# patngnw/NewsRecommendation

Measured on AMD Instinct MI355X. Metric: train impressions/sec @ batch 512, NRMS, higher is better.
Workload: dtype bf16; 1 GPU; NRMS train step (fwd+bwd+Adam), MIND-small shapes: title_len=30, history=50, npratio=4, 300-d word table; per_gpu_batch=512, global_batch=512, vocab_rows=30000, freeze_embedding=False, compact_history=False, dense_batch=False, feed=resident, deterministic=False, optimizer=flat bucket + HIP fused Adam, parallelism=dp1

## Files before the change

include/nrhip.h:

```cpp
#ifndef NRHIP_H
#define NRHIP_H

#include <stddef.h>
#include <stdint.h>

#ifdef __cplusplus
extern "C" {
#endif

#define NR_F32 0
#define NR_BF16 1

#define NR_OK 0
#define NR_ERR_ARG 1
#define NR_ERR_HIP 2

#define NR_SRC_DENSE 0
#define NR_SRC_GATHER 1

typedef void* nr_stream_t;

int nr_version(void);
int nr_last_error(char* buf, size_t n);
int nr_abi_sizes(size_t* out, int n);
int nr_set_deterministic(void* scratch, size_t bytes);
int nr_set_option(const char* name, int value);
int nr_get_option(const char* name);


int nr_cast_pad(const float* src, int rows, int cols, int ld_src, void* dst, int ld_dst, int dtype,
                int transpose, nr_stream_t stream);
#define NR_CAST_BATCH_MAX 16
typedef struct {
  const float* src;
  void* dst;
  int rows, cols, ld_src, ld_dst, transpose;
} nr_cast_job;
int nr_cast_pad_batch(const nr_cast_job* jobs, int n, int dtype, nr_stream_t stream);
int nr_pack_conv_w(const float* w, int N, int D, void* dst, int Dp, int dtype, nr_stream_t stream);
int nr_unpack_conv_dw(const float* dw_pack, int N, int D, int Dp, float* dw, int accumulate, nr_stream_t stream);
int nr_pack_conv_w_t(const float* w, int N, int D, void* dst, int ld, int dtype, nr_stream_t stream);

int nr_embed_gather_fwd(const void* table, int ld_table, int dtype, const int32_t* ids, int n_ids,
                        int ids_stride, int cols, float* out, int ld_out, nr_stream_t stream);
int nr_embed_gather_bwd(const float* dout, int ld_dout, const int32_t* ids, int n_ids, int ids_stride,
                        int cols, float* dtable, int ld_dtable, nr_stream_t stream);
int nr_gather_cast_fwd(const float* table, int ld_table, const int32_t* ids, int n_ids, int cols, void* out, int ld_out,
                       int out_dtype, nr_stream_t stream);

typedef struct {
  int n, L, d_model, heads, d_head, dtype;
  int src_kind;
  const void* x;
  int ldx;
  const int32_t* ids;
  float p_in;
  uint32_t seed_in;
  float p_out;
  uint32_t seed_out;
  const float* mask;
  const void* w_qkv;
  int ldw;
  const float* b_qkv;
  void* x_rows;
  int ld_rows;
  int32_t* row_ws;
  size_t row_ws_bytes;
  int table_rows;
  const void* proj_table;
  const int32_t* seq_needed;
  const int32_t* seq_nz;
  int row_ws_ready;
  int bwd_phase;
  int y_far_unwritten;
  int dy_far_unwritten;
} nr_mhsa_desc;

int nr_mhsa_fwd_fused(const nr_mhsa_desc* d);
int nr_mhsa_compact_rows(const nr_mhsa_desc* d);
size_t nr_mhsa_workspace_bytes(const nr_mhsa_desc* d);
int nr_mhsa_fwd(const nr_mhsa_desc* d, void* qkv, void* y, nr_stream_t stream);
int nr_mhsa_bwd(const nr_mhsa_desc* d, const void* qkv, const void* dy, void* dqkv, const void* w_qkv_t,
                int ldwt, float* dw_qkv, float* db_qkv, void* dx, float* dtable, nr_stream_t stream);

int nr_sdpa_fwd(const void* qkv, const float* mask, void* y, int n, int L, int heads, int d_head, int dtype, float p_out,
                uint32_t seed_out, nr_stream_t stream);
int nr_sdpa_bwd(const void* qkv, const float* mask, const void* dy, void* dqkv, int n, int L, int heads, int d_head,
                int dtype, float p_out, uint32_t seed_out, nr_stream_t stream);

int nr_sdpa_long_fwd(const void* qkv, const float* mask, void* y, int n, int L, int heads, int d_head, int dtype, float p_out,
                     uint32_t seed_out, nr_stream_t stream);
int nr_sdpa_long_bwd(const void* qkv, const float* mask, const void* dy, void* dqkv, int n, int L, int heads, int d_head,
                     int dtype, float p_out, uint32_t seed_out, nr_stream_t stream);

int nr_check_ids(const int32_t* ids, int count, int stride, int rows, int32_t* bad, nr_stream_t stream);
int nr_check_labels(const int64_t* label, int count, int classes, int32_t* bad, nr_stream_t stream);

typedef struct {
  int n, T, D, Dp, N, dtype;
  const void* table;
  const int32_t* ids;
  int ids_stride;
  float p_in;
  uint32_t seed_in;
  const void* w_pack;
  const float* bias;
  void* x_rows;
  int ld_rows;
  int32_t* bwd_ws;
  size_t bwd_ws_bytes;
  const int32_t* seq_nz;
  const int32_t* seq_needed;
  int table_rows;
} nr_conv_desc;
size_t nr_conv_workspace_bytes(const nr_conv_desc* d);
int nr_conv1d_k3_fwd(const nr_conv_desc* d, void* y, nr_stream_t stream);
int nr_conv1d_k3_bwd(const nr_conv_desc* d, const void* dy, float* dw_pack, float* db, nr_stream_t stream);
size_t nr_conv_table_workspace_bytes(const nr_conv_desc* d);
int nr_conv1d_k3_bwd_table(const nr_conv_desc* d, const void* dy, const void* w_t_pack, int ldwt, float* dtable, void* ws, size_t ws_bytes,
                           nr_stream_t stream);

typedef struct {
  int n, L, N, q, dtype;
  const void* x;
  const float* mask;
  const void* w1;
  int ldw1;
  const float* b1;
  const float* w2;
  const float* b2;
  size_t partial_bytes;
  const int32_t* seq_needed;
  int dx_far_unwritten;
} nr_pool_desc;
int nr_pool_contracts_slabs(const nr_pool_desc* d);
size_t nr_pool_workspace_bytes(const nr_pool_desc* d);
const int32_t* nr_pool_seq_flags(const nr_pool_desc* d, const float* partial);
int nr_additive_pool_fwd(const nr_pool_desc* d, void* e, float* alpha, float* out, int ld_out, nr_stream_t stream);
int nr_additive_pool_bwd(const nr_pool_desc* d, const void* e, const float* alpha, const float* g, int ld_g,
                         const void* w1_t, int ldw1t, void* dpre, float* partial, float* dw1, float* db1,
                         float* dw2, float* db2, void* dx, nr_stream_t stream);

int nr_pad_blend_fwd(const float* x, const float* mask, const float* pad, void* out, int n, int L, int N,
                     int dtype, nr_stream_t stream);
int nr_pad_blend_bwd(const void* dout, const float* mask, float* dx, float* dpad, int n, int L, int N,
                     int dtype, nr_stream_t stream);

typedef struct {
  int M, K, N, dtype;
  int src_kind;
  const void* x;
  int ldx;
  const int32_t* ids;
  int ids_stride;
  const void* w;
  int ldw;
  const float* bias;
  const void* w_t;
  int ldwt;
  size_t dout_ws_bytes;
  int table_rows;
} nr_linear_desc;
size_t nr_linear_workspace_bytes(const nr_linear_desc* d);
int nr_linear_fwd(const nr_linear_desc* d, float* out, int ld_out, nr_stream_t stream);
int nr_linear_bwd(const nr_linear_desc* d, const float* dout, int ld_dout, void* dout_ws, float* dw,
                  float* db, float* dtable, nr_stream_t stream);

int nr_score_ce_fwd(const float* cand, int ld_cand, const float* user, const int64_t* label, float* score,
                    float* loss, float* lossvec, int B, int C, int N, nr_stream_t stream);
int nr_score_ce_bwd(const float* cand, int ld_cand, const float* user, const int64_t* label,
                    const float* score, const float* gloss, const float* gscore, float* dcand, int ld_dcand,
                    float* duser, int B, int C, int N, nr_stream_t stream);
int nr_score_eval(const float* news_vecs, int ld_news, const int32_t* cand_ids, const int32_t* imp_of,
                  const float* user, int ld_user, float* score, int n_cand, int N, nr_stream_t stream);

#define NR_TOPK_MAX_K 128
#define NR_TOPK_MAX_N 1024
#define NR_TOPK_MAX_EXCLUDE 64
typedef struct {
  const float* news_vecs;
  int ld_news, V;
  const float* user;
  int ld_user, U;
  int N, k;
  const int32_t* exclude;
  int ld_exclude, E;
  const int32_t* excl_offsets;
// ... 527 lines not shown
```

newsrecommendation_amd/_lib.py:

```python
from __future__ import annotations

import ctypes as C
import os
import subprocess
import threading

NR_F32, NR_BF16 = 0, 1
NR_SRC_DENSE, NR_SRC_GATHER = 0, 1

_HERE = os.path.dirname(os.path.abspath(__file__))
LIB_PATH = os.environ.get("NRHIP_LIB") or os.path.join(_HERE, "libnrhip.so")
CSRC_DIR = os.path.join(_HERE, "csrc")

c_f32p = C.POINTER(C.c_float)
c_i32p = C.POINTER(C.c_int32)
c_i64p = C.POINTER(C.c_int64)


class MhsaDesc(C.Structure):
    _fields_ = [("n", C.c_int), ("L", C.c_int), ("d_model", C.c_int), ("heads", C.c_int), ("d_head", C.c_int),
                ("dtype", C.c_int), ("src_kind", C.c_int), ("x", C.c_void_p), ("ldx", C.c_int), ("ids", C.c_void_p),
                ("p_in", C.c_float), ("seed_in", C.c_uint32), ("p_out", C.c_float), ("seed_out", C.c_uint32),
                ("mask", C.c_void_p), ("w_qkv", C.c_void_p), ("ldw", C.c_int), ("b_qkv", C.c_void_p),
                ("x_rows", C.c_void_p), ("ld_rows", C.c_int), ("row_ws", C.c_void_p), ("row_ws_bytes", C.c_size_t),
                ("table_rows", C.c_int), ("proj_table", C.c_void_p), ("seq_needed", C.c_void_p), ("seq_nz", C.c_void_p), ("row_ws_ready", C.c_int), ("bwd_phase", C.c_int),
                ("y_far_unwritten", C.c_int), ("dy_far_unwritten", C.c_int)]


class ConvDesc(C.Structure):
    _fields_ = [("n", C.c_int), ("T", C.c_int), ("D", C.c_int), ("Dp", C.c_int), ("N", C.c_int), ("dtype", C.c_int),
                ("table", C.c_void_p), ("ids", C.c_void_p), ("ids_stride", C.c_int), ("p_in", C.c_float),
                ("seed_in", C.c_uint32), ("w_pack", C.c_void_p), ("bias", C.c_void_p), ("x_rows", C.c_void_p),
                ("ld_rows", C.c_int), ("bwd_ws", C.c_void_p), ("bwd_ws_bytes", C.c_size_t), ("seq_nz", C.c_void_p),
                ("seq_needed", C.c_void_p), ("table_rows", C.c_int)]


CAST_BATCH_MAX = 16


class CastJob(C.Structure):
    _fields_ = [("src", C.c_void_p), ("dst", C.c_void_p), ("rows", C.c_int), ("cols", C.c_int), ("ld_src", C.c_int),
                ("ld_dst", C.c_int), ("transpose", C.c_int)]


class PackJob(C.Structure):
    _fields_ = [("first", C.c_size_t), ("count", C.c_size_t), ("cols", C.c_int), ("ld_dst", C.c_int), ("dst", C.c_void_p)]


ADAM_PACK_MAX = 4


class AdamRowsDesc(C.Structure):
    _fields_ = [("param", C.c_void_p), ("grad", C.c_void_p), ("exp_avg", C.c_void_p), ("exp_avg_sq", C.c_void_p), ("rows", C.c_int),
                ("width", C.c_int), ("row_step", C.c_void_p), ("sched", C.c_void_p), ("sched_capacity", C.c_int), ("ids", C.c_void_p),
                ("ids_stride", C.c_int), ("n_ids", C.c_int), ("upto", C.c_int), ("apply", C.c_int), ("zero_grad", C.c_int),
                ("lr", C.c_float), ("beta1", C.c_float), ("beta2", C.c_float), ("eps", C.c_float), ("grad_scale", C.c_float),
                ("pack_dst", C.c_void_p), ("pack_cols", C.c_int), ("pack_ld", C.c_int), ("ws", C.c_void_p), ("ws_bytes", C.c_size_t)]


NR_TOPK_MAX_K, NR_TOPK_MAX_N, NR_TOPK_MAX_EXCLUDE = 128, 1024, 64


class TopkDesc(C.Structure):
    _fields_ = [("news_vecs", C.c_void_p), ("ld_news", C.c_int), ("V", C.c_int), ("user", C.c_void_p), ("ld_user", C.c_int), ("U", C.c_int),
                ("N", C.c_int), ("k", C.c_int), ("exclude", C.c_void_p), ("ld_exclude", C.c_int), ("E", C.c_int),
                ("excl_offsets", C.c_void_p), ("excl_ids", C.c_void_p), ("n_excl", C.c_int), ("splits", C.c_int),
                ("group", C.c_void_p), ("group_cap", C.c_int),
                ("out_ids", C.c_void_p), ("out_scores", C.c_void_p), ("ws", C.c_void_p), ("ws_bytes", C.c_size_t),
                ("prior", C.c_void_p), ("stamp", C.c_void_p), ("window", C.c_void_p), ("ld_window", C.c_int)]


NR_RANK_MAX_TARGETS, NR_RANK_MAX_KS = 64, 8
NR_RANK_MAX_GROUPS, NR_RANK_MAX_CAPPED_TARGETS = 512, 4


class RankDesc(C.Structure):
    _fields_ = [("news_vecs", C.c_void_p), ("ld_news", C.c_int), ("V", C.c_int), ("user", C.c_void_p), ("ld_user", C.c_int), ("U", C.c_int),
                ("N", C.c_int), ("T", C.c_int), ("targets", C.c_void_p), ("ld_targets", C.c_int), ("exclude", C.c_void_p),
                ("ld_exclude", C.c_int), ("E", C.c_int), ("excl_offsets", C.c_void_p), ("excl_ids", C.c_void_p), ("n_excl", C.c_int),
# ... 81 lines not shown
                ("sub_ids", C.c_void_p), ("sub_w", C.c_void_p), ("ld_sub", C.c_int), ("T", C.c_int), ("scale_inv_tau", C.c_int),
                ("out", C.c_void_p), ("ld_out", C.c_int), ("out_mass", C.c_void_p), ("ws", C.c_void_p), ("ws_bytes", C.c_size_t),
                ("prior", C.c_void_p), ("stamp", C.c_void_p), ("window", C.c_void_p), ("ld_window", C.c_int)]


class LogprobCappedGradDesc(C.Structure):
    _fields_ = [("news_vecs", C.c_void_p), ("ld_news", C.c_int), ("V", C.c_int), ("user", C.c_void_p), ("ld_user", C.c_int), ("U", C.c_int),
                ("N", C.c_int), ("k", C.c_int), ("row_ids", C.c_void_p), ("ld_ids", C.c_int), ("group", C.c_void_p), ("group_cap", C.c_int),
                ("n_groups", C.c_int), ("tau", C.c_float), ("tau_u", C.c_void_p), ("base_max", C.c_void_p), ("base_logsum", C.c_void_p),
                ("ld_base", C.c_int), ("g", C.c_void_p), ("ld_g", C.c_int), ("out_bin_w", C.c_void_p), ("out_sub_w", C.c_void_p),
                ("prior", C.c_void_p), ("stamp", C.c_void_p), ("window", C.c_void_p), ("ld_window", C.c_int)]


class ExpectNewsGroupsDesc(C.Structure):
    _fields_ = [("news_vecs", C.c_void_p), ("ld_news", C.c_int), ("V", C.c_int), ("user", C.c_void_p), ("ld_user", C.c_int), ("U", C.c_int),
                ("N", C.c_int), ("splits", C.c_int), ("excl_offsets", C.c_void_p), ("excl_users", C.c_void_p), ("n_excl", C.c_int),
                ("tau", C.c_float), ("tau_u", C.c_void_p), ("order", C.c_void_p), ("n_pos", C.c_int), ("bin_start", C.c_void_p),
                ("n_groups", C.c_int), ("base_max", C.c_void_p), ("base_logsum", C.c_void_p), ("bin_w", C.c_void_p), ("ld_bin", C.c_int),
                ("scale_inv_tau", C.c_int), ("named_offsets", C.c_void_p), ("named_user", C.c_void_p), ("named_w", C.c_void_p),
                ("n_named", C.c_int), ("out", C.c_void_p), ("ld_out", C.c_int), ("out_mass", C.c_void_p), ("ws", C.c_void_p),
                ("ws_bytes", C.c_size_t), ("prior", C.c_void_p), ("stamp", C.c_void_p), ("window", C.c_void_p), ("ld_window", C.c_int)]


class EntropyDesc(C.Structure):
    _fields_ = [("news_vecs", C.c_void_p), ("ld_news", C.c_int), ("V", C.c_int), ("user", C.c_void_p), ("ld_user", C.c_int), ("U", C.c_int),
                ("N", C.c_int), ("splits", C.c_int), ("excl_offsets", C.c_void_p), ("excl_ids", C.c_void_p), ("n_excl", C.c_int),
                ("tau", C.c_float), ("tau_u", C.c_void_p), ("base_max", C.c_void_p), ("base_logsum", C.c_void_p),
                ("out_entropy", C.c_void_p), ("out_var", C.c_void_p), ("out_mass", C.c_void_p), ("ws", C.c_void_p), ("ws_bytes", C.c_size_t),
                ("prior", C.c_void_p), ("stamp", C.c_void_p), ("window", C.c_void_p), ("ld_window", C.c_int)]


class ExpectAffineDesc(C.Structure):
    _fields_ = [("news_vecs", C.c_void_p), ("ld_news", C.c_int), ("V", C.c_int), ("user", C.c_void_p), ("ld_user", C.c_int), ("U", C.c_int),
                ("N", C.c_int), ("splits", C.c_int), ("excl_offsets", C.c_void_p), ("excl_ids", C.c_void_p), ("n_excl", C.c_int),
                ("tau", C.c_float), ("tau_u", C.c_void_p), ("base_max", C.c_void_p), ("base_logsum", C.c_void_p), ("alpha", C.c_void_p),
                ("beta", C.c_void_p), ("sub_ids", C.c_void_p), ("sub_w", C.c_void_p), ("ld_sub", C.c_int), ("T", C.c_int),
                ("scale_inv_tau", C.c_int), ("out", C.c_void_p), ("ld_out", C.c_int), ("out_mass", C.c_void_p), ("ws", C.c_void_p),
                ("ws_bytes", C.c_size_t), ("prior", C.c_void_p), ("stamp", C.c_void_p), ("window", C.c_void_p), ("ld_window", C.c_int)]


class ExpectNewsAffineDesc(C.Structure):
    _fields_ = [("news_vecs", C.c_void_p), ("ld_news", C.c_int), ("V", C.c_int), ("user", C.c_void_p), ("ld_user", C.c_int), ("U", C.c_int),
                ("N", C.c_int), ("splits", C.c_int), ("excl_offsets", C.c_void_p), ("excl_users", C.c_void_p), ("n_excl", C.c_int),
                ("tau", C.c_float), ("tau_u", C.c_void_p), ("base_max", C.c_void_p), ("base_logsum", C.c_void_p), ("alpha", C.c_void_p),
                ("beta", C.c_void_p), ("scale_inv_tau", C.c_int), ("named_offsets", C.c_void_p), ("named_user", C.c_void_p),
                ("named_w", C.c_void_p), ("n_named", C.c_int), ("out", C.c_void_p), ("ld_out", C.c_int), ("out_mass", C.c_void_p),
                ("ws", C.c_void_p), ("ws_bytes", C.c_size_t), ("prior", C.c_void_p), ("stamp", C.c_void_p), ("window", C.c_void_p),
                ("ld_window", C.c_int)]


class PoolDesc(C.Structure):
    _fields_ = [("n", C.c_int), ("L", C.c_int), ("N", C.c_int), ("q", C.c_int), ("dtype", C.c_int), ("x", C.c_void_p),
                ("mask", C.c_void_p), ("w1", C.c_void_p), ("ldw1", C.c_int), ("b1", C.c_void_p), ("w2", C.c_void_p),
                ("b2", C.c_void_p), ("partial_bytes", C.c_size_t), ("seq_needed", C.c_void_p), ("dx_far_unwritten", C.c_int)]


class LinearDesc(C.Structure):
    _fields_ = [("M", C.c_int), ("K", C.c_int), ("N", C.c_int), ("dtype", C.c_int), ("src_kind", C.c_int),
                ("x", C.c_void_p), ("ldx", C.c_int), ("ids", C.c_void_p), ("ids_stride", C.c_int), ("w", C.c_void_p),
                ("ldw", C.c_int), ("bias", C.c_void_p), ("w_t", C.c_void_p), ("ldwt", C.c_int), ("dout_ws_bytes", C.c_size_t), ("table_rows", C.c_int)]


_vp, _i, _f, _u32 = C.c_void_p, C.c_int, C.c_float, C.c_uint32
RESTYPES = {"nr_pool_seq_flags": C.c_void_p, "nr_eval_metrics_workspace_bytes": C.c_size_t, "nr_mhsa_workspace_bytes": C.c_size_t, "nr_conv_workspace_bytes": C.c_size_t, "nr_conv_table_workspace_bytes": C.c_size_t, "nr_pool_workspace_bytes": C.c_size_t,
            "nr_linear_workspace_bytes": C.c_size_t, "nr_adam_rows_workspace_bytes": C.c_size_t,
            "nr_score_topk_workspace_bytes": C.c_size_t, "nr_score_rank_workspace_bytes": C.c_size_t,
            "nr_score_sample_workspace_bytes": C.c_size_t, "nr_score_logz_workspace_bytes": C.c_size_t,
            "nr_score_logz_groups_workspace_bytes": C.c_size_t, "nr_score_expect_workspace_bytes": C.c_size_t,
            "nr_score_expect_news_workspace_bytes": C.c_size_t, "nr_score_expect_groups_workspace_bytes": C.c_size_t,
            "nr_score_expect_news_groups_workspace_bytes": C.c_size_t, "nr_score_entropy_workspace_bytes": C.c_size_t,
            "nr_score_expect_affine_workspace_bytes": C.c_size_t, "nr_score_expect_news_affine_workspace_bytes": C.c_size_t}
SIGNATURES = {
    "nr_version": [],
    "nr_last_error": [C.c_char_p, C.c_size_t],
    "nr_abi_sizes": [C.POINTER(C.c_size_t), _i],
    "nr_set_deterministic": [_vp, C.c_size_t],
    "nr_set_option": [C.c_char_p, _i],
    "nr_get_option": [C.c_char_p],
    "nr_mhsa_workspace_bytes": [C.POINTER(MhsaDesc)],
    "nr_conv_workspace_bytes": [C.POINTER(ConvDesc)],
    "nr_conv_table_workspace_bytes": [C.POINTER(ConvDesc)],
    "nr_pool_workspace_bytes": [C.POINTER(PoolDesc)],
    "nr_pool_contracts_slabs": [C.POINTER(PoolDesc)],
    "nr_pool_seq_flags": [C.POINTER(PoolDesc), _vp],
    "nr_linear_workspace_bytes": [C.POINTER(LinearDesc)],
    "nr_sdpa_fwd": [_vp, _vp, _vp, _i, _i, _i, _i, _i, _f, _u32, _vp],
    "nr_sdpa_bwd": [_vp, _vp, _vp, _vp, _i, _i, _i, _i, _i, _f, _u32, _vp],
    "nr_sdpa_long_fwd": [_vp, _vp, _vp, _i, _i, _i, _i, _i, _f, _u32, _vp],
    "nr_sdpa_long_bwd": [_vp, _vp, _vp, _vp, _i, _i, _i, _i, _i, _f, _u32, _vp],
    "nr_assemble_batch": [_vp, _i, _i, _vp, _vp, _vp, _vp, _i, _i, _i, _vp, _vp, _vp, _vp],
    "nr_stack_rows": [_vp, _i, _vp, _i, _i, _vp, _vp, _vp, _vp],
    "nr_eval_metrics_workspace_bytes": [_i],
    "nr_eval_metrics": [_vp, _vp, _vp, _i, _i, _vp, C.c_size_t, _vp, _vp],
    "nr_adam_step": [_vp, _vp, _vp, _vp, C.c_size_t, _f, _f, _f, _f, _i, _f, _i, _vp],
    "nr_adam_step_packed": [_vp, _vp, _vp, _vp, C.c_size_t, _f, _f, _f, _f, _i, _f, _i, _vp, _i, _vp],
    "nr_adam_rows_workspace_bytes": [_i],
    "nr_adam_rows": [C.POINTER(AdamRowsDesc), _vp],
    "nr_check_ids": [_vp, _i, _i, _i, _vp, _vp],
    "nr_check_labels": [_vp, _i, _i, _vp, _vp],
    "nr_cast_pad": [_vp, _i, _i, _i, _vp, _i, _i, _i, _vp],
    "nr_cast_pad_batch": [_vp, _i, _i, _vp],
    "nr_pack_conv_w": [_vp, _i, _i, _vp, _i, _i, _vp],
    "nr_unpack_conv_dw": [_vp, _i, _i, _i, _vp, _i, _vp],
    "nr_pack_conv_w_t": [_vp, _i, _i, _vp, _i, _i, _vp],
    "nr_embed_gather_fwd": [_vp, _i, _i, _vp, _i, _i, _i, _vp, _i, _vp],
    "nr_embed_gather_bwd": [_vp, _i, _vp, _i, _i, _i, _vp, _i, _vp],
    "nr_gather_cast_fwd": [_vp, _i, _vp, _i, _i, _vp, _i, _i, _vp],
    "nr_mhsa_fwd_fused": [C.POINTER(MhsaDesc)],
    "nr_mhsa_compact_rows": [C.POINTER(MhsaDesc)],
    "nr_mhsa_fwd": [C.POINTER(MhsaDesc), _vp, _vp, _vp],
    "nr_mhsa_bwd": [C.POINTER(MhsaDesc), _vp, _vp, _vp, _vp, _i, _vp, _vp, _vp, _vp, _vp],
    "nr_conv1d_k3_fwd": [C.POINTER(ConvDesc), _vp, _vp],
    "nr_conv1d_k3_bwd": [C.POINTER(ConvDesc), _vp, _vp, _vp, _vp],
    "nr_conv1d_k3_bwd_table": [C.POINTER(ConvDesc), _vp, _vp, _i, _vp, _vp, C.c_size_t, _vp],
    "nr_additive_pool_fwd": [C.POINTER(PoolDesc), _vp, _vp, _vp, _i, _vp],
    "nr_additive_pool_bwd": [C.POINTER(PoolDesc), _vp, _vp, _vp, _i, _vp, _i, _vp, _vp, _vp, _vp, _vp, _vp, _vp, _vp],
    "nr_pad_blend_fwd": [_vp, _vp, _vp, _vp, _i, _i, _i, _i, _vp],
    "nr_pad_blend_bwd": [_vp, _vp, _vp, _vp, _i, _i, _i, _i, _vp],
    "nr_linear_fwd": [C.POINTER(LinearDesc), _vp, _i, _vp],
    "nr_linear_bwd": [C.POINTER(LinearDesc), _vp, _i, _vp, _vp, _vp, _vp, _vp],
    "nr_score_ce_fwd": [_vp, _i, _vp, _vp, _vp, _vp, _vp, _i, _i, _i, _vp],
    "nr_score_ce_bwd": [_vp, _i, _vp, _vp, _vp, _vp, _vp, _vp, _i, _vp, _i, _i, _i, _vp],
    "nr_score_eval": [_vp, _i, _vp, _vp, _vp, _i, _vp, _i, _i, _vp],
    "nr_score_topk_workspace_bytes": [C.POINTER(TopkDesc)],
    "nr_score_topk": [C.POINTER(TopkDesc), _vp],
    "nr_score_rank_workspace_bytes": [C.POINTER(RankDesc)],
    "nr_score_rank": [C.POINTER(RankDesc), _vp],
    "nr_mmr_select": [C.POINTER(MmrDesc), _vp],
    "nr_score_sample_workspace_bytes": [C.POINTER(SampleDesc)],
    "nr_score_sample": [C.POINTER(SampleDesc), _vp],
    "nr_sample_noise": [C.c_uint64, _u32, _vp, _vp, _i, _vp, _vp, _vp],
    "nr_score_logz_workspace_bytes": [C.POINTER(LogzDesc)],
    "nr_score_logz": [C.POINTER(LogzDesc), _vp],
    "nr_row_logprob": [C.POINTER(LogprobDesc), _vp],
    "nr_score_logz_groups_workspace_bytes": [C.POINTER(LogzGroupsDesc)],
    "nr_score_logz_groups": [C.POINTER(LogzGroupsDesc), _vp],
# ... 113 lines not shown
```

newsrecommendation_amd/csrc/nr_api.hip:

```cpp
#include <stdarg.h>
#include <stdio.h>
#include <stdlib.h>
#include <string.h>

#include "nr_gemm.h"

int nr_launch_attn(bool bwd, int dtype, const void* qkv, const float* mask, void* y, const void* dy, void* dqkv, int n, int L,
                   int heads, int d_head, const DropCfg& drop, hipStream_t stream, const uint32_t* tmask = nullptr,
                   const float* bias = nullptr, const int32_t* seq_list = nullptr, const int32_t* seq_count = nullptr,
                   const int32_t* needed = nullptr);
bool nr_attn_pad_ok(int dtype, int L, int d_head, const void* p0, const void* p1);
bool nr_attn_rowsub_ok(int dtype, int L, int d_head, int heads);
bool nr_attn_compact_ok(int dtype, int L, int d_head, int heads);
int nr_launch_attn_bwd_compact(const void* qkv, const float* mask, const void* dy, void* dqkv, int n, int L, int heads, int d_head,
                               const DropCfg& drop, hipStream_t stream, const uint32_t* tmask, const float* bias, const int32_t* seq_list,
                               const int32_t* seq_count, const int32_t* pos, void* dump, float* db, const int32_t* nzf);
int nr_launch_attn_gather_fwd(const void* proj_table, const int32_t* ids, const float* mask, void* y, int n, int L, int heads,
                              int d_head, const DropCfg& drop, hipStream_t stream);
int nr_launch_pool_core_fwd(int dtype, const void* x, const void* e, const float* w2, const float* b2, const float* mask,
                            float* alpha, float* out, int ld_out, int n, int L, int N, int q, hipStream_t s,
                            const int32_t* needed = nullptr);
int nr_launch_pool_core_bwd(int dtype, const void* x, const void* e, const float* w2, const float* alpha, const float* g,
                            int ld_g, void* dpre, float* partial, float* dw2, float* db2, int n, int L, int N, int q,
                            hipStream_t s, const int32_t* seq_nz = nullptr);
// ... 423 lines not shown
  if (n >= 14) out[13] = sizeof(nr_logz_groups_desc);
  if (n >= 15) out[14] = sizeof(nr_logprob_capped_desc);
  if (n >= 16) out[15] = sizeof(nr_expect_desc);
  if (n >= 17) out[16] = sizeof(nr_expect_news_desc);
  if (n >= 18) out[17] = sizeof(nr_logprob_grad_desc);
  if (n >= 20) { out[18] = sizeof(nr_expect_groups_desc); out[19] = sizeof(nr_logprob_capped_grad_desc); }
  if (n >= 21) out[20] = sizeof(nr_expect_news_groups_desc);
  if (n >= 23) { out[21] = sizeof(nr_entropy_desc); out[22] = sizeof(nr_expect_affine_desc); }
  if (n >= 24) out[23] = sizeof(nr_expect_news_affine_desc);
  return NR_OK;
}

int nr_set_deterministic(void* scratch, size_t bytes) {
  NR_CHECK_ARG(scratch == nullptr || (bytes >= 8 && (((uintptr_t)scratch) & 7) == 0), "set_deterministic: scratch must be 8-byte aligned and non-empty");
  g_det_elems.store(scratch ? bytes / 8 : 0);
  g_det_ws.store(reinterpret_cast<long long*>(scratch));
  return NR_OK;
}

int nr_set_option(const char* name, int value) {
  NR_CHECK_ARG(name != nullptr, "set_option: null name");
  (void)nr_opt(0);
  if (strncmp(name, "NR_", 3) == 0) name += 3;
  for (int i = 0; i < NR_OPT_COUNT; ++i)
    if (strcmp(name, g_opt_defs[i].name) == 0) {
      g_opt[i].store(value, std::memory_order_relaxed);
      return NR_OK;
    }
  nr_set_error("set_option: unknown option %s", name);
  return NR_ERR_ARG;
}

int nr_get_option(const char* name) {
  if (name == nullptr) return -1;
  if (strncmp(name, "NR_", 3) == 0) name += 3;
  for (int i = 0; i < NR_OPT_COUNT; ++i)
    if (strcmp(name, g_opt_defs[i].name) == 0) return nr_opt(i);
  return -1;
}

size_t nr_mhsa_workspace_bytes(const nr_mhsa_desc* d) {
  return (d == nullptr || d->n < 0 || d->L < 1) ? 0 : mhsa_ws_of(d).total * sizeof(int32_t);
}
size_t nr_conv_workspace_bytes(const nr_conv_desc* d) {
  return (d == nullptr || d->n < 0 || d->T < 1) ? 0 : conv_ws_elems(d->n, d->T) * sizeof(int32_t);
}
size_t nr_conv_table_workspace_bytes(const nr_conv_desc* d) {
  if (d == nullptr || d->n < 0 || d->T < 1 || d->D < 1 || d->N < 1 || d->table_rows < 1 || !dtype_ok(d->dtype)) return 0;
  return conv_tab_layout(d->n, d->T, d->D, d->N, d->table_rows, d->dtype).total;
}
int nr_pool_contracts_slabs(const nr_pool_desc* d) {
  return (d != nullptr && d->n > 0 && d->L >= 1 && d->q >= 1 && dtype_ok(d->dtype) && pool_has_flags(d)) ? 1 : 0;
}
size_t nr_pool_workspace_bytes(const nr_pool_desc* d) {
  return (d == nullptr || d->n < 0 || d->L < 1 || d->q < 1) ? 0 : pool_ws_elems(d->n, d->L, d->q, d->N, d->dtype) * sizeof(float);
}
const int32_t* nr_pool_seq_flags(const nr_pool_desc* d, const float* partial) {
  if (d == nullptr || partial == nullptr || d->n <= 0 || d->L < 1 || d->q < 1 || !dtype_ok(d->dtype) || !pool_has_flags(d)) return nullptr;
  return reinterpret_cast<const int32_t*>(partial + pool_ws_used(d->n, d->q));
}
size_t nr_linear_workspace_bytes(const nr_linear_desc* d) {
  if (d == nullptr || d->M < 0 || d->N < 1 || !dtype_ok(d->dtype)) return 0;
  return (size_t)d->M * round_up(d->N, nr_chunk(d->dtype)) * nr_elt_size(d->dtype);
}

namespace {
__global__ __launch_bounds__(256) void check_ids_kernel(const int32_t* __restrict__ ids, int count, int stride, int rows,
                                                        int32_t* __restrict__ bad) {
  int nbad = 0;
  for (long i = (long)blockIdx.x * 256 + threadIdx.x; i < count; i += (long)gridDim.x * 256) {
    const int v = ids[i * stride];
    nbad += (v < 0 || v >= rows) ? 1 : 0;
  }
  nbad = (int)wave_sum((float)nbad);
  if ((threadIdx.x & 63) == 0 && nbad) atomicAdd(bad, nbad);
}
__global__ __launch_bounds__(256) void check_labels_kernel(const int64_t* __restrict__ label, int count, int classes,
                                                           int32_t* __restrict__ bad) {
  int nbad = 0;
  for (long i = (long)blockIdx.x * 256 + threadIdx.x; i < count; i += (long)gridDim.x * 256) {
    const int64_t v = label[i];
    nbad += (v < 0 || v >= classes) ? 1 : 0;
  }
  nbad = (int)wave_sum((float)nbad);
  if ((threadIdx.x & 63) == 0 && nbad) atomicAdd(bad, nbad);
}
}

int nr_check_ids(const int32_t* ids, int count, int stride, int rows, int32_t* bad, nr_stream_t stream) {
  NR_CHECK_ARG(count >= 0 && stride >= 1 && rows >= 0 && bad != nullptr && (count == 0 || ids != nullptr), "check_ids: bad arguments");
  if (count == 0) return NR_OK;
  NR_DEVICE_GUARD(stream, bad);
  const int blocks = count / 256 + 1 > 1024 ? 1024 : count / 256 + 1;
  hipLaunchKernelGGL(check_ids_kernel, dim3(blocks), dim3(256), 0, (hipStream_t)stream, ids, count, stride, rows, bad);
  NR_CHECK_LAUNCH();
  return NR_OK;
}

int nr_check_labels(const int64_t* label, int count, int classes, int32_t* bad, nr_stream_t stream) {
  NR_CHECK_ARG(count >= 0 && classes >= 0 && bad != nullptr && (count == 0 || label != nullptr), "check_labels: bad arguments");
  if (count == 0) return NR_OK;
  NR_DEVICE_GUARD(stream, bad);
  const int blocks = count / 256 + 1 > 1024 ? 1024 : count / 256 + 1;
  hipLaunchKernelGGL(check_labels_kernel, dim3(blocks), dim3(256), 0, (hipStream_t)stream, label, count, classes, bad);
  NR_CHECK_LAUNCH();
  return NR_OK;
// ... 51 lines not shown
int nr_sdpa_long_bwd(const void* qkv, const float* mask, const void* dy, void* dqkv, int n, int L, int heads, int d_head, int dtype,
                     float p_out, uint32_t seed_out, nr_stream_t stream) {
  int rc = sdpa_long_check(qkv, n, L, heads, d_head, dtype, p_out);
  if (rc) return rc;
  if (n == 0) return NR_OK;
  NR_CHECK_ARG(dy != nullptr && dqkv != nullptr, "sdpa_long_bwd: null operand");
  NR_DEVICE_GUARD(stream, dqkv);
  return nr_launch_attn(true, dtype, qkv, mask, nullptr, dy, dqkv, n, L, heads, d_head, nr_make_drop(p_out, seed_out), (hipStream_t)stream);
}

int nr_gemm_nt(int dtype, const void* A, int lda, const void* B, int ldb, const float* bias, int act_tanh, void* C, int ldc,
               int out_dtype, int M, int N, int K, nr_stream_t stream) {
  NR_CHECK_ARG(dtype_ok(dtype) && dtype_ok(out_dtype) && A && B && C, "gemm_nt: bad dtype / null operand");
  NR_DEVICE_GUARD(stream, C);
  RowSrc a = dense_rows(A, lda, K);
  EpiArgs ep = store_epi(C, ldc, out_dtype, bias, act_tanh);
  return nr_launch_gemm_nt(dtype, a, B, ldb, M, N, K, EPI_STORE, ep, (hipStream_t)stream);
}

int nr_gemm_tn(int dtype, const void* dC, int ldc, const void* A, int lda, float* dW, int ldw, float* db, int M, int N, int K,
               nr_stream_t stream) {
  NR_CHECK_ARG(dtype_ok(dtype) && dC && A && dW, "gemm_tn: bad dtype / null operand");
  NR_DEVICE_GUARD(stream, dW);
  RowSrc a = dense_rows(A, lda, K);
  DetScope det((hipStream_t)stream);
  if (det.on() && M > 0 && N > 0 && K > 0 && ldw >= K) {
    det.add(dW, (size_t)(N - 1) * ldw + K);
    det.add(db, (size_t)N);
    int rc = det.begin(true, false);
    if (rc) return rc;
  }
  return nr_launch_gemm_tn(dtype, dC, ldc, a, dW, ldw, db, M, N, K, N, K, (hipStream_t)stream);
}

int nr_mhsa_fwd_fused(const nr_mhsa_desc* d) {
  if (d == nullptr) return 0;
  return d->dtype == NR_BF16 && d->src_kind == NR_SRC_GATHER && (((uintptr_t)d->x | (uintptr_t)d->w_qkv) & 15) == 0 &&
                 nr_mhsa_fused_shape_ok(d->L, d->heads, d->d_head, d->d_model, d->ldx, d->ldw)
             ? 1
             : 0;
}

int nr_mhsa_compact_rows(const nr_mhsa_desc* d) {
  MhsaPlan P;
  return (d != nullptr && mhsa_check(d, &P) == NR_OK && P.compact_rows) ? 1 : 0;
}

int nr_mhsa_fwd(const nr_mhsa_desc* d, void* qkv, void* y, nr_stream_t stream) {
  MhsaPlan P;
  int rc = mhsa_check(d, &P);
  if (rc) return rc;
  if (d->n == 0) return NR_OK;
  NR_CHECK_ARG(y != nullptr, "mhsa_fwd: null output");
  hipStream_t s = (hipStream_t)stream;
  NR_DEVICE_GUARD(stream, y);
  const int N = d->heads * d->d_head, M = P.M, Kp = P.Kp;
  const MhsaWs W = mhsa_ws_of(d);
  RowSrc A;
  if ((rc = mhsa_rows(d, &A))) return rc;
  if (d->proj_table != nullptr) {
    NR_CHECK_ARG(d->src_kind == NR_SRC_GATHER && d->p_in == 0.f && d->dtype == NR_BF16 && d->ids != nullptr && qkv == nullptr,
                 "mhsa_fwd: proj_table needs a bf16 gather source without input dropout and no qkv buffer (no backward)");
    rc = nr_launch_attn_gather_fwd(d->proj_table, d->ids, d->mask, y, d->n, d->L, d->heads, d->d_head, nr_make_drop(d->p_out, d->seed_out), s);
    NR_CHECK_ARG(rc >= 0, "mhsa_fwd: proj_table is only supported for L <= 64, d_head %% 4 == 0 (<= 32), 8-byte aligned tensors");
    return rc;
  }
  if (qkv == nullptr && d->dtype == NR_BF16 && d->src_kind == NR_SRC_GATHER) {
    rc = nr_launch_mhsa_fused_fwd(d->x, d->ldx, d->ids, d->w_qkv, d->ldw, d->b_qkv, d->mask, nullptr, d->x_rows, d->ld_rows, y, d->n,
                                  d->L, d->heads, d->d_head, d->d_model, nr_make_drop(d->p_in, d->seed_in),
                                  nr_make_drop(d->p_out, d->seed_out), s);
    if (rc >= 0) return rc;
  }
  NR_CHECK_ARG(qkv != nullptr, "mhsa_fwd: the unfused path needs the qkv buffer (see nr_mhsa_fwd_fused)");
  EpiArgs ep = store_epi(qkv, 3 * N, d->dtype, d->b_qkv, 0);
  const uint32_t* tmask = nullptr;
  int32_t* ws = d->row_ws;
  if (P.keeps_rows) {
    NR_CHECK_ARG(d->ld_rows >= Kp && d->ld_rows % nr_chunk(d->dtype) == 0, "mhsa_fwd: ld_rows=%d must cover %d", d->ld_rows, Kp);
    if (P.compacts && (rc = nr_launch_compact_rows_fwd(d->ids, M, d->n, d->L, d->x, d->d_model, ws, s, P.compact_rows ? ws + W.pos : nullptr,
                                                       ws + W.seq, P.compact_rows ? ws + W.hist : nullptr, d->table_rows)))
      return rc;
    if (P.compacts) { ep.row_count = ws; ep.row_idx = ws + W.live_idx; ep.row_ids = ws + W.live_ids; }
  }
  if (P.compact_rows) {
    NR_CHECK_ARG(aligned(8, qkv, y), "mhsa_fwd: qkv / y must be 8-byte aligned");
    if ((rc = nr_launch_gather_live_rows(d->dtype, A, d->x_rows, d->ld_rows, M, Kp, ws, ws + W.live_idx, ws + W.live_ids, s,
                                         ws + W.hist, d->table_rows)))
      return rc;
    A = dense_rows(d->x_rows, d->ld_rows, d->d_model);
    ep.a_dense = 1;
    tmask = reinterpret_cast<const uint32_t*>(ws + W.tmask);
  } else if (P.keeps_rows) {
    if ((rc = nr_launch_rows_materialize(d->dtype, A, d->x_rows, d->ld_rows, M, Kp, s, P.skip_far ? d->seq_needed : nullptr, 32 / d->L + 2,
                                         d->L, P.skip_far ? ws + 2 : nullptr)))
      return rc;
    A = dense_rows(d->x_rows, d->ld_rows, d->d_model);
    if (P.pad_sub && aligned(8, qkv, y)) tmask = reinterpret_cast<const uint32_t*>(ws + W.tmask);
    if (P.compacts && !(tmask != nullptr && P.row_sub) &&
        (rc = nr_launch_bias_rows(qkv, 3 * N, 3 * N, d->b_qkv, ws + W.dead_idx, ws + 1, M, tmask, d->L, s)))
      return rc;
  }
  if ((rc = nr_launch_gemm_nt(d->dtype, A, d->w_qkv, d->ldw, M, 3 * N, Kp, EPI_STORE, ep, s))) return rc;
  const int32_t* fwd_list = nullptr;
  if (P.needed_list && tmask != nullptr && aligned(16, y)) {
    int32_t* lw = ws + W.seq;
    if ((rc = nr_launch_needed_list(d->seq_needed, d->n, lw, y, (size_t)d->L * N * nr_elt_size(d->dtype), s,
                                    d->y_far_unwritten ? 32 / d->L + 2 : -1, true)))
      return rc;
    fwd_list = lw;
  }
  return nr_launch_attn(false, d->dtype, qkv, d->mask, y, nullptr, nullptr, d->n, d->L, d->heads, d->d_head,
                        nr_make_drop(d->p_out, d->seed_out), s, tmask, tmask ? d->b_qkv : nullptr, fwd_list ? fwd_list + 4 : nullptr, fwd_list,
                        fwd_list ? nullptr : d->seq_needed);
}

static int mhsa_bwd_compact(const nr_mhsa_desc* d, const MhsaPlan& P, const uint32_t* tmask, const void* qkv, const void* dy, void* dqkv,
                            const void* w_qkv_t, int ldwt, float* dw_qkv, float* db_qkv, void* dx, float* dtable, hipStream_t s) {
  int rc = NR_OK;
  const int N = d->heads * d->d_head, M = P.M;
  const MhsaWs W = mhsa_ws_of(d);
  NR_CHECK_ARG(tmask != nullptr, "mhsa_bwd: the forward stored x_rows compactly; qkv / dy / dqkv must be 8-byte aligned");
  NR_CHECK_ARG(!d->dy_far_unwritten || d->seq_nz != nullptr, "mhsa_bwd: dy_far_unwritten needs the seq_nz flags");
  NR_CHECK_ARG(dx == nullptr && (dtable == nullptr || (w_qkv_t != nullptr && ldwt >= 3 * N)),
               "mhsa_bwd: gather source takes dtable or nothing, not dx (and with dtable, w_qkv_t [d_model, >=3N])");
  int32_t* ws = d->row_ws;
  if (d->bwd_phase != 2) {
    const int32_t* flags = d->seq_nz;
    if (flags == nullptr) {
      if ((rc = nr_launch_title_flags(dy, d->n, d->L, N, ws + W.slab, s))) return rc;
      flags = ws + W.slab;
    }
    int32_t* seq_ws = ws + W.seq;
    if ((rc = nr_launch_zero_tail_rows(dqkv, 3 * N, ws, M, s, seq_ws, 4))) return rc;
    if ((rc = nr_launch_seq_list(flags, tmask, d->n, d->L, seq_ws, s, 0, true))) return rc;
    if ((rc = nr_launch_attn_bwd_compact(qkv, d->mask, dy, dqkv, d->n, d->L, d->heads, d->d_head, nr_make_drop(d->p_out, d->seed_out), s, tmask,
                                         d->b_qkv, seq_ws + 4, seq_ws, ws + W.pos, ws + W.dump, db_qkv, d->dy_far_unwritten ? flags : nullptr)))
      return rc;
    if (dtable != nullptr) {
      if ((rc = nr_launch_sort_rows_by_id(ws, ws + W.live_idx, ws + W.live_ids, M, d->table_rows, ws + W.hist, ws + W.sort_idx, ws + W.sort_ids, s,
                                          ws + W.sort_k, ws + W.cursor)))
        return rc;
      EpiArgs ep = store_epi(dtable, d->d_model, NR_F32, nullptr, 0);
      ep.ids = d->ids; ep.ids_stride = 1; ep.Dtrue = d->d_model; ep.drop = nr_make_drop(d->p_in, d->seed_in);
      ep.row_count = ws; ep.row_idx = ws + W.sort_idx; ep.row_ids = ws + W.sort_ids; ep.a_idx = ws + W.sort_k;
      RowSrc G = dense_rows(dqkv, 3 * N, 3 * N);
      if ((rc = nr_launch_gemm_nt(d->dtype, G, w_qkv_t, ldwt, M, d->d_model, 3 * N, EPI_SCATTER, ep, s))) return rc;
    }
  }
  if (d->bwd_phase != 1)
    rc = nr_launch_gemm_tn_counted(dqkv, 3 * N, d->x_rows, d->ld_rows, dw_qkv, d->d_model, M, 3 * N, P.Kp, 3 * N, d->d_model, ws, s,
                                   W.tn_floats ? reinterpret_cast<float*>(ws + W.tn_scratch) : nullptr, W.tn_floats);
  return rc;
}

static int mhsa_bwd_rows(const nr_mhsa_desc* d, const MhsaPlan& P, const uint32_t* tmask, const RowSrc& A, const void* qkv, const void* dy,
                         void* dqkv, const void* w_qkv_t, int ldwt, float* dw_qkv, float* db_qkv, void* dx, float* dtable, hipStream_t s) {
  int rc = NR_OK;
  const int N = d->heads * d->d_head, M = P.M, Kp = P.Kp;
  const MhsaWs W = mhsa_ws_of(d);
  const bool ph_main = d->bwd_phase != 2;
// ... 167 lines not shown
               d->D, d->N);
  NR_CHECK_ARG(d->table_rows >= 1, "conv1d_bwd_table: table_rows=%d (rows V of the table) is required", d->table_rows);
  NR_CHECK_ARG((uint64_t)d->table_rows * (uint64_t)d->T < 0x7fffffffull, "conv1d_bwd_table: table_rows * T = %llu does not fit 31 bits",
               (unsigned long long)d->table_rows * (unsigned long long)d->T);
  NR_CHECK_ARG((uint64_t)d->n * d->T * (uint64_t)(d->D > d->N ? d->D : d->N) < 0xffffffffull,
               "conv1d_bwd_table: problem too large for 32-bit element counters");
  NR_CHECK_ARG(d->p_in >= 0.f && d->p_in < 1.f, "conv1d_bwd_table: dropout p out of range");
  if (d->n == 0) return NR_OK;
  NR_CHECK_ARG(d->ids && d->ids_stride >= 1 && dy && w_t_pack && dtable && ws, "conv1d_bwd_table: null operand");
  NR_CHECK_ARG(ldwt >= 3 * d->N && ldwt % ch == 0, "conv1d_bwd_table: w_t_pack is [D, ldwt >= 3N] (ldwt=%d, N=%d)", ldwt, d->N);
  const ConvTabWs W = conv_tab_layout(d->n, d->T, d->D, d->N, d->table_rows, d->dtype);
  NR_CHECK_ARG(ws_bytes >= W.total, "conv1d_bwd_table: ws holds %zu bytes, nr_conv_table_workspace_bytes() asks for %zu", ws_bytes, W.total);
  NR_CHECK_ARG(aligned(16, dy, ws, w_t_pack) && aligned(4, dtable), "conv1d_bwd_table: dy / w_t_pack / ws must be 16-byte aligned");
  NR_DEVICE_GUARD(stream, dtable);
  hipStream_t s = (hipStream_t)stream;
  int32_t* wi = static_cast<int32_t*>(ws);
  void* dyg = static_cast<char*>(ws) + W.dyg;
  void* dx = static_cast<char*>(ws) + W.dx;
  const int n = d->n, T = d->T, N = d->N, D = d->D, V = d->table_rows, K = 3 * N;
  const bool compact = d->dtype == NR_BF16 && K >= 192 && ldwt >= (K + 31) / 32 * 32;
  int rc;
  if ((rc = nr_launch_conv_table_live(d->ids, d->ids_stride, d->seq_nz, n, T, V, wi, wi + W.live_s, wi + W.live_id, s))) return rc;
  if ((rc = nr_launch_conv_table_stage(d->dtype, dy, n, T, N, wi, wi + W.live_s, compact, dyg, compact ? wi + W.ident : nullptr, s))) return rc;
  RowSrc A = dense_rows(dyg, N, K);
  A.gap = T;
  EpiArgs ep = store_epi(dx, W.Dc, d->dtype, nullptr, 0);
  if (compact) { ep.row_count = wi + 1; ep.row_idx = wi + W.ident; }
  if ((rc = nr_launch_gemm_nt(d->dtype, A, w_t_pack, ldwt, n * T, D, K, EPI_STORE, ep, s))) return rc;
  if ((rc = nr_launch_sort_rows_by_id(wi, wi + W.live_s, wi + W.live_id, n, V, wi + W.hist, wi + W.sort_s, wi + W.sort_id, s, wi + W.sort_k)))
    return rc;
  if ((rc = nr_launch_conv_table_rank(wi, wi + W.sort_s, wi + W.sort_id, wi + W.sort_k, wi + W.hist, compact, n, wi + W.ord_s, wi + W.ord_slot, s)))
    return rc;
  return nr_launch_conv_table_scatter(d->dtype, dx, W.Dc, n, T, D, V, wi, wi + W.sort_id, wi + W.hist, wi + W.ord_s, wi + W.ord_slot,
                                      nr_make_drop(d->p_in, d->seed_in), dtable, s);
}

static int pool_check(const nr_pool_desc* d) {
  NR_CHECK_ARG(d != nullptr, "additive_pool: null descriptor");
  NR_CHECK_ARG(dtype_ok(d->dtype), "additive_pool: bad dtype %d", d->dtype);
  const int ch = nr_chunk(d->dtype);
  NR_CHECK_ARG(d->n >= 0 && d->L >= 1 && d->L <= 128 && d->N >= 1 && d->q >= 1, "additive_pool: bad shape n=%d L=%d N=%d q=%d", d->n, d->L,
               d->N, d->q);
  NR_CHECK_ARG(d->N % ch == 0 && d->q % ch == 0, "additive_pool: N=%d and q=%d must be multiples of %d for this dtype", d->N, d->q, ch);
  NR_CHECK_ARG(d->ldw1 >= d->N, "additive_pool: ldw1=%d < N=%d", d->ldw1, d->N);
  NR_CHECK_ARG(d->n == 0 || (d->x && d->w1 && d->b1 && d->w2 && d->b2), "additive_pool: null operand");
  return NR_OK;
}

int nr_additive_pool_fwd(const nr_pool_desc* d, void* e, float* alpha, float* out, int ld_out, nr_stream_t stream) {
  int rc = pool_check(d);
  if (rc) return rc;
  if (d->n == 0) return NR_OK;
  NR_CHECK_ARG(e && alpha && out && ld_out >= d->N, "additive_pool_fwd: null output / ld_out");
  NR_DEVICE_GUARD(stream, out);
  hipStream_t s = (hipStream_t)stream;
  if (nr_pool_fused_fwd_ok(d->dtype, d->n, d->L, d->N, d->q, d->ldw1) && ((((uintptr_t)d->x) | ((uintptr_t)d->w1) | ((uintptr_t)e)) & 15) == 0 &&
      d->N % 8 == 0 && d->mask == nullptr)
    return nr_launch_pool_fused_fwd(d->x, d->N, d->w1, d->ldw1, d->b1, d->w2, d->b2, d->mask, e, d->q, alpha, out, ld_out, d->n, d->L, d->N, d->q,
                                    d->seq_needed, s);
  RowSrc A = dense_rows(d->x, d->N, d->N);
  EpiArgs ep = store_epi(e, d->q, d->dtype, d->b1, 1);
  ep.seq_nz = d->seq_needed; ep.L = d->L;
  if ((rc = nr_launch_gemm_nt(d->dtype, A, d->w1, d->ldw1, d->n * d->L, d->q, d->N, EPI_STORE, ep, s))) return rc;
  return nr_launch_pool_core_fwd(d->dtype, d->x, e, d->w2, d->b2, d->mask, alpha, out, ld_out, d->n, d->L, d->N, d->q, s, d->seq_needed);
}

int nr_additive_pool_bwd(const nr_pool_desc* d, const void* e, const float* alpha, const float* g, int ld_g, const void* w1_t,
                         int ldw1t, void* dpre, float* partial, float* dw1, float* db1, float* dw2, float* db2, void* dx,
                         nr_stream_t stream) {
  int rc = pool_check(d);
  if (rc) return rc;
  if (d->n == 0) return NR_OK;
  NR_CHECK_ARG(e && alpha && g && dpre && partial && dw1 && db1 && dw2 && db2, "additive_pool_bwd: null operand");
  NR_DEVICE_GUARD(stream, dpre);
  NR_CHECK_ARG(d->partial_bytes >= pool_ws_elems(d->n, d->L, d->q, d->N, d->dtype) * sizeof(float),
               "additive_pool_bwd: partial holds %zu bytes, nr_pool_workspace_bytes() asks for %zu", d->partial_bytes,
               pool_ws_elems(d->n, d->L, d->q, d->N, d->dtype) * sizeof(float));
  float* tn_scratch = partial + pool_ws_ints(d->n, d->L, d->q);
  const size_t tn_floats = pool_tn_floats(d->n, d->L, d->q, d->N, d->dtype);
  hipStream_t s = (hipStream_t)stream;
  const int M = d->n * d->L;
  DetScope det(s);
  det.add(dw1, (size_t)d->q * d->N);
  det.add(db1, (size_t)d->q);
  det.add(dw2, (size_t)d->q);
  det.add(db2, 1);
  if ((rc = det.begin(true, true))) return rc;
  int32_t* ws = nullptr;
  if (pool_has_flags(d)) {
    ws = reinterpret_cast<int32_t*>(partial + pool_ws_used(d->n, d->q));
    if ((rc = nr_launch_row_flags_f32(g, ld_g, d->N, d->n, ws, s))) return rc;
  }
  const int32_t* zero_flags = ws != nullptr ? ws : d->seq_needed;
  if (ws != nullptr && dx != nullptr && w1_t != nullptr && !det.on() && nr_pool_fused_bwd_ok(d->dtype, d->n, d->L, d->N, d->q, ldw1t) && ld_g % 4 == 0 &&
      ((((uintptr_t)d->x) | ((uintptr_t)e) | ((uintptr_t)w1_t) | ((uintptr_t)dpre) | ((uintptr_t)dx) | ((uintptr_t)g)) & 15) == 0 && d->N % 8 == 0) {
    int rows = 0;
    if ((rc = nr_launch_pool_fused_bwd(d->x, d->N, e, d->q, alpha, g, ld_g, d->w2, w1_t, ldw1t, dpre, d->q, dx, d->N, partial,
                                       nr_pool_partial_rows(d->n), ws, d->n, d->L, d->N, d->q, s, &rows, d->dx_far_unwritten)))
      return rc;
    if ((rc = nr_launch_colsum_split(partial, rows, d->q + 1, d->q + 1, dw2, d->q, db2, s))) return rc;
    if ((rc = nr_launch_live_slabs(ws, d->n, d->L, s))) return rc;
    return gemm_tn_live_slabs(ws, d->n, dpre, d->q, d->x, d->N, dw1, d->N, db1, M, d->q, d->N, d->q, d->N, s, 0, tn_scratch, tn_floats);
  }
  if ((rc = nr_launch_pool_core_bwd(d->dtype, d->x, e, d->w2, alpha, g, ld_g, dpre, partial, dw2, db2, d->n, d->L, d->N, d->q, s, zero_flags)))
    return rc;
  RowSrc X = dense_rows(d->x, d->N, d->N);
  if (ws != nullptr) {
    if ((rc = nr_launch_live_slabs(ws, d->n, d->L, s))) return rc;
    if ((rc = gemm_tn_live_slabs(ws, d->n, dpre, d->q, d->x, d->N, dw1, d->N, db1, M, d->q, d->N, d->q, d->N, s, 0, tn_scratch, tn_floats))) return rc;
  } else if ((rc = nr_launch_gemm_tn(d->dtype, dpre, d->q, X, dw1, d->N, db1, M, d->q, d->N, d->q, d->N, s))) {
    return rc;
  }
// ... 76 lines not shown
```

newsrecommendation_amd/csrc/nr_gemm.h:

```cpp
#pragma once
#include "nr_common.h"

enum { ROWS_DENSE = 0, ROWS_GATHER = 1, ROWS_IM2COL3 = 2 };

struct RowSrc {
  const void* base;
  const int32_t* ids;
  int ld;
  int ids_stride;
  int kind;
  int Tlen;
  int Dtrue;
  DropCfg drop;
  int gap;
};

enum {
  EPI_STORE = 0,
  EPI_POOLBWD = 1,
  EPI_SCATTER = 2,
  EPI_STORE_TANH = 3,
};

struct EpiArgs {
  void* C;
  int ldc;
  int out_dtype;
  const float* bias;
  int act_tanh;
  const float* rowscale;
  const float* G;
  int ldg, L;
  const int32_t* ids;
  int ids_stride;
  int Dtrue;
  DropCfg drop;
  const int32_t* row_count;
  const int32_t* row_idx;
  const int32_t* row_ids;
  const int32_t* seq_nz;
  void* rows_out;
  int ld_rows_out;
  int a_gap;
  const int32_t* a_idx;
  int a_dense;
  int tail_cus;
};

int nr_launch_gemm_nt(int dtype, const RowSrc& A, const void* B, int ldb, int M, int N, int K, int epi,
                      const EpiArgs& ep, hipStream_t stream);
int nr_launch_conv_rows(int dtype, const RowSrc& A, void* out, int n, hipStream_t stream, const int32_t* needed = nullptr, int margin = 0);
int nr_launch_rows_materialize(int dtype, const RowSrc& A, void* out, int ldo, int M, int K, hipStream_t stream,
                               const int32_t* needed = nullptr, int margin = 0, int L = 0, const int32_t* keep_all = nullptr);
int nr_launch_compact_rows(const int32_t* ids, int ids_stride, int M, int32_t* ws, hipStream_t stream);
int nr_launch_sort_rows_by_id(const int32_t* count, const int32_t* rows, const int32_t* ids, int Mmax, int table_rows, int32_t* hist,
                              int32_t* rows_out, int32_t* ids_out, hipStream_t stream, int32_t* k_out = nullptr,
                              int32_t* counted_cursor = nullptr);
int nr_launch_compact_rows_fwd(const int32_t* ids, int M, int n, int L, const void* table_row0, int cols, int32_t* ws,
                               hipStream_t stream, int32_t* posmap = nullptr, int32_t* zero4 = nullptr, int32_t* zhist = nullptr,
                               int nhist = 0);
int nr_launch_bias_rows(void* C, int ldc, int N, const float* bias, const int32_t* rows, const int32_t* count, int max_rows,
                        const uint32_t* tmask, int L, hipStream_t stream);
int nr_launch_title_flags(const void* dy, int n, int L, int N, int32_t* title_nz, hipStream_t stream);
int nr_launch_row_flags_f32(const float* g, int ld, int N, int n, int32_t* nz, hipStream_t stream);
int nr_launch_live_slabs(int32_t* ws, int n, int L, hipStream_t stream);
int nr_launch_needed_list(const int32_t* flags, int n, int32_t* out, void* y, size_t seq_bytes, hipStream_t stream, int reach = -1,
                          bool zeroed = false);
int nr_launch_seq_list(const int32_t* title_nz, const uint32_t* tmask, int n, int L, int32_t* out, hipStream_t stream, int reach = -1,
                       bool zeroed = false);
int nr_launch_zero_tail_rows(void* buf, int ld, const int32_t* count, int Mmax, hipStream_t stream, int32_t* za = nullptr, int na = 0,
                             int32_t* zb = nullptr, int nb = 0);
int nr_launch_gemm_tn_slabs(const void* dC, int ldc, const void* X, int ldx, float* dW, int ldw, float* db, int M, int N, int K,
                            int Nstore, int Kstore, const int32_t* slab_list, const int32_t* slab_count, hipStream_t stream, int xgap = 0,
                            float* scratch = nullptr, size_t scratch_floats = 0);
size_t nr_gemm_tn_scratch_floats(int M, int N, int K);
bool nr_gemm_tn_slabs_ok(int ldc, int ldx, int M, int N, int K);
int nr_pool_fused_fwd_ok(int dtype, int n, int L, int N, int q, int ldw1);
int nr_launch_pool_fused_fwd(const void* x, int ldx, const void* w1, int ldw1, const float* b1, const float* w2, const float* b2,
                             const float* mask, void* e, int lde, float* alpha, float* out, int ld_out, int n, int L, int N, int q,
                             const int32_t* needed, hipStream_t stream);
int nr_launch_gemm_tn_counted(const void* dC, int ldc, const void* X, int ldx, float* dW, int ldw, int Mmax, int N, int K, int Nstore,
                              int Kstore, const int32_t* row_count, hipStream_t stream, float* scratch = nullptr, size_t scratch_floats = 0);
int nr_pool_fused_bwd_ok(int dtype, int n, int L, int N, int q, int ldw1t);
int nr_launch_pool_fused_bwd(const void* x, int ldx, const void* e, int lde, const float* alpha, const float* g, int ldg, const float* w2,
                             const void* w1t, int ldw1t, void* dpre, int ldp, void* dx, int lddx, float* partial, int partial_rows,
                             const int32_t* nz, int n, int L, int N, int q, hipStream_t stream, int* grid_out, int dx_far_unwritten = 0);
int nr_launch_gather_live_rows(int dtype, const RowSrc& A, void* out, int ldo, int Mmax, int K, const int32_t* count, const int32_t* rows,
                               const int32_t* ids, hipStream_t stream, int32_t* hist = nullptr, int V = 0);
int nr_launch_gemm_tn(int dtype, const void* dC, int ldc, const RowSrc& A, float* dW, int ldw, float* db,
                      int M, int N, int K, int Nstore, int Kstore, hipStream_t stream);
int nr_launch_conv_table_live(const int32_t* ids, int ids_stride, const int32_t* seq_nz, int n, int T, int V, int32_t* hdr, int32_t* live_s,
                              int32_t* live_id, hipStream_t stream);
int nr_launch_conv_table_stage(int dtype, const void* dy, int n, int T, int N, const int32_t* hdr, const int32_t* live_s, bool compact, void* out,
                               int32_t* ident, hipStream_t stream);
int nr_launch_conv_table_rank(const int32_t* hdr, const int32_t* sort_s, const int32_t* sort_id, const int32_t* sort_k, const int32_t* cursor,
                              bool compact, int n, int32_t* ord_s, int32_t* ord_slot, hipStream_t stream);
int nr_launch_conv_table_scatter(int dx_dtype, const void* dx, int ldx, int n, int T, int D, int V, const int32_t* hdr, const int32_t* sort_id,
                                 const int32_t* cursor, const int32_t* ord_s, const int32_t* ord_slot, DropCfg drop, float* dtable,
                                 hipStream_t stream);
```

newsrecommendation_amd/csrc/nr_gemm.hip:

```cpp
#include <stdlib.h>

#include "nr_gemm.h"
#include "nr_scatter_tail.h"

namespace {

constexpr int BM = 128, BN = 128, BK = 32, NTHR = 256;
constexpr int SC = BN + 4;

template <typename T> struct TileCfg {
  static constexpr int CH = 16 / (int)sizeof(T);
  static constexpr int SK = BK + CH;
  static constexpr int CPR = BK / CH;
  static constexpr int NCH = BM * CPR / NTHR;
  static constexpr int RPC = BM / CH;
  static constexpr size_t STAGE_BYTES = (size_t)2 * 2 * BM * SK * sizeof(T);
};
constexpr size_t EPI_BYTES = (size_t)64 * SC * sizeof(float);

template <typename T> constexpr size_t smem_bytes() {
  return TileCfg<T>::STAGE_BYTES > EPI_BYTES ? TileCfg<T>::STAGE_BYTES : EPI_BYTES;
}

union Chunk {
// ... 1613 lines not shown
  };
  for (int i = i0; i < i1; i += U) {
    uint64_t bal[U];
    ballots(i, bal);
#pragma unroll
    for (int u = 0; u < U; ++u) {
      if (i + u < i1) {
        if (i + u - i0 == lane) mybal = bal[u];
        cnt += __popcll(bal[u]);
      }
    }
  }
  if (lane == 0) sCnt[wid] = cnt;
  __syncthreads();
  int rank = 0, total = 0;
#pragma unroll
  for (int w = 0; w < NW; ++w) {
    const int cw = sCnt[w];
    rank += w < wid ? cw : 0;
    total += cw;
  }
  for (int g0 = i0; g0 < i1; g0 += KEPT) {
    uint64_t gb = mybal;
    if (g0 != i0) {
      gb = 0;
#pragma unroll 1
      for (int k = 0; k < KEPT; k += U) {
        uint64_t bal[U];
        ballots(g0 + k, bal);
#pragma unroll
        for (int u = 0; u < U; ++u)
          if (g0 + k + u < i1 && k + u == lane) gb = bal[u];
      }
    }
    const int c = __popcll(gb);
    int incl = c;
#pragma unroll
    for (int d = 1; d < 64; d <<= 1) {
      const int t = __shfl_up(incl, d, 64);
      if (lane >= d) incl += t;
    }
    const int lo = rank + incl - c, hi = rank + incl;
    int q = lo <= b0 ? 0 : (lo - b0 + G - 1) / G;
    for (int t = b0 + q * G; t < hi; t += G, ++q) {
      uint64_t w = gb;
      for (int z = t - lo; z > 0; --z) w &= w - 1;
      sList[q] = (g0 + lane) * 64 + (__ffsll((unsigned long long)w) - 1);
    }
    rank += __shfl(incl, 63, 64);
  }
  return b0 < total ? (total - b0 + G - 1) / G : 0;
}

struct PoolFusedArgs {
  const bf16_t* x; int ldx;
  const bf16_t* w1; int ldw1;
  const float* b1; const float* w2; const float* b2;
  bf16_t* e; int lde;
  float* alpha;
  float* out; int ld_out;
  const int32_t* needed;
  int n, L, N, q;
};

template <int KS>
struct PoolFusedCfg {
  static constexpr int NW = 8, TPW = 2, RT = 2, R = 32;
  static constexpr int APIECES = RT * KS, PW = (APIECES + NW - 1) / NW, STAGE = APIECES * 1024;
  static constexpr int NS = 4;
  static constexpr int S = RT;
  static constexpr int NCOL = KS * 32;
  static constexpr int DUMP = NS * STAGE, BIAS = DUMP + NW * 1024;
  static constexpr int PART = BIAS + 1024;
  static constexpr int RED = PART + 2 * NW * 32 * 4;
  static constexpr int LIST = RED + 2 * NW * NCOL * 4;
  static constexpr int STEADY = PW + 2 * (S + 2);
  static_assert(STEADY <= 62, "vmcnt is a 6-bit counter");
};

template <int KS>
__global__ __launch_bounds__(512) void pool_fused_fwd_kernel(PoolFusedArgs a, int max_steps) {
  using Cfg = PoolFusedCfg<KS>;
  constexpr int NW = Cfg::NW, TPW = Cfg::TPW, RT = Cfg::RT, R = Cfg::R, NS = Cfg::NS, PW = Cfg::PW, STAGE = Cfg::STAGE, NCOL = Cfg::NCOL;
  constexpr int APIECES = Cfg::APIECES;
  extern __shared__ __attribute__((aligned(16))) char smem[];
  const uint32_t lds0 = (uint32_t)(size_t)(__attribute__((address_space(3))) char*)smem;
  const int tid = threadIdx.x, lane = tid & 63;
  const int wid = __builtin_amdgcn_readfirstlane(tid >> 6);
  const int fr = lane & 15, g = lane >> 4;
  const int prow = lane >> 2, c8 = ((lane & 3) ^ swzP(prow)) * 8;
  const int L = a.L, N = a.N, q = a.q, M = a.n * a.L;
  float* sBias = reinterpret_cast<float*>(smem + Cfg::BIAS);
  float* sPart = reinterpret_cast<float*>(smem + Cfg::PART);
  float* sRed = reinterpret_cast<float*>(smem + Cfg::RED);
  int* sList = reinterpret_cast<int*>(smem + Cfg::LIST);

  const int G = gridDim.x, b0 = blockIdx.x;
  int nsteps = b0 < a.n ? (a.n - b0 + G - 1) / G : 0;
  if (a.needed != nullptr) {
    __shared__ int sCnt[NW + 1];
    const int cand = nsteps;
    const int run = pool_balanced_walk<NW>(a.needed, a.n, G, b0, sList, sCnt, wid, lane);
    for (int c = wid; c < cand; c += NW) {
      const int sq = b0 + c * G;
      if (a.needed[sq] != 0) continue;
      if (lane < L) a.alpha[(size_t)sq * L + lane] = 0.f;
      for (int col = lane; col < N; col += 64) a.out[(size_t)sq * a.ld_out + col] = 0.f;
    }
    nsteps = run;
  } else {
    for (int c = tid; c < nsteps; c += 512) sList[c] = b0 + c * G;
  }
  if (nsteps == 0) return;

  const int wcol0 = wid * TPW * 16;
  bf16x8 bfr[TPW][KS];
  float w2r[TPW][4];
#pragma unroll
  for (int t = 0; t < TPW; ++t) {
    const int nrow = min(wcol0 + t * 16 + fr, q - 1);
    const bf16_t* brow = a.w1 + (size_t)nrow * a.ldw1 + 8 * g;
#pragma unroll
    for (int s2 = 0; s2 < KS; ++s2) bfr[t][s2] = *reinterpret_cast<const bf16x8*>(brow + 32 * s2);
#pragma unroll
    for (int r = 0; r < 4; ++r) {
      const int col = wcol0 + t * 16 + 4 * g + r;
      w2r[t][r] = col < q ? a.w2[col] : 0.f;
    }
  }
  for (int c = tid; c < NW * TPW * 16; c += 512) sBias[c] = c < q ? a.b1[c] : 0.f;
  const float b2 = a.b2[0];
  __builtin_amdgcn_s_waitcnt(0x0F70);
  __syncthreads();

  const uint32_t dump_lds = lds0 + Cfg::DUMP + wid * 1024;
  auto issue_stage = [&](int kk) {
    const uint32_t slot = lds0 + (kk % NS) * STAGE;
    const bool real = kk < nsteps;
    const int row0 = real ? sList[kk] * L : 0;
    const bf16_t* rowp[RT];
#pragma unroll
    for (int i = 0; i < RT; ++i) rowp[i] = a.x + (size_t)min(row0 + 16 * i + prow, M - 1) * a.ldx + c8;
#pragma unroll
    for (int u = 0; u < PW; ++u) {
      const int p = wid + NW * u;
      if (real && p < APIECES) {
        const int i = p / KS, s2 = p - i * KS;
        const bf16_t* rp = i == 0 ? rowp[0] : rowp[1];
        dma16(rp + min(32 * s2, N - 8 - c8), slot + p * 1024);
      } else {
        dma16(a.x + c8, dump_lds);
      }
    }
  };
  uint4* dump_g = g_nt_dump + wid * 64 + lane;
  const int offA = fr * 64 + ((g ^ swzP(fr)) << 4);
  const int cc = lane, ccp = cc >> 2, ccs = cc & 3;
  const bool cc_ok = cc * 8 < N;

#pragma unroll 1
  for (int kk = 0; kk < NS - 2; ++kk) issue_stage(kk);

  auto sum32 = [&](float v) {
    v += __builtin_bit_cast(float, __builtin_amdgcn_update_dpp(0, __builtin_bit_cast(int, v), 0x128, 0xf, 0xf, false));
    v += __builtin_bit_cast(float, __builtin_amdgcn_update_dpp(0, __builtin_bit_cast(int, v), 0x124, 0xf, 0xf, false));
    v += __builtin_bit_cast(float, __builtin_amdgcn_update_dpp(0, __builtin_bit_cast(int, v), 0x122, 0xf, 0xf, false));
    v += __builtin_bit_cast(float, __builtin_amdgcn_update_dpp(0, __builtin_bit_cast(int, v), 0x121, 0xf, 0xf, false));
    return v + __shfl_xor(v, 16, 64);
  };
  auto phase_out = [&](int k) {
    const int kf = k - 2;
    float* dst = reinterpret_cast<float*>(dump_g);
    if (kf >= 0 && kf < nsteps && tid < N) {
      const float* red = sRed + (kf & 1) * NW * NCOL + tid;
      float v = 0.f;
#pragma unroll
      for (int r = 0; r < NW; ++r) v += red[r * NCOL];
      *(a.out + (size_t)sList[kf] * a.ld_out + tid) = v;
    } else {
      *dst = 0.f;
    }
  };
  auto phase_alpha = [&](int k) {
    const int kp = k - 1;
    const bool real = kp >= 0 && kp < nsteps;
    const int sq = real ? sList[kp] : 0;
    const float* part = sPart + (kp & 1) * NW * 32 + (lane & 31);
    float sl = b2;
#pragma unroll
    for (int w = 0; w < NW; ++w) sl += part[w * 32];
    const float ex = (lane & 31) < L ? __expf(sl) : 0.f;
    const float al = ex / (sum32(ex) + 1e-8f);
    float* adst = (real && wid == 0 && lane < L) ? a.alpha + (size_t)sq * L + lane : reinterpret_cast<float*>(dump_g);
    *adst = al;
    if (real) {
      const char* st = smem + (kp % NS) * STAGE;
      const int ccr = cc_ok ? cc : 0;
      bf16x8 xv[R / NW];
#pragma unroll
      for (int j = 0; j < R / NW; ++j) {
        const int m = min(wid + NW * j, L - 1);
        xv[j] = *reinterpret_cast<const bf16x8*>(st + ((m >> 4) * KS + (ccr >> 2)) * 1024 + (m & 15) * 64 + (((ccr & 3) ^ swzP(m & 15)) << 4));
      }
      float acc[8];
#pragma unroll
      for (int e2 = 0; e2 < 8; ++e2) acc[e2] = 0.f;
#pragma unroll
      for (int j = 0; j < R / NW; ++j) {
// ... 13 lines not shown
    const bool real = k < nsteps;
    const int row0 = real ? sList[k] * L : 0;
    const char* st = smem + (k % NS) * STAGE;
    f32x4 acc[RT][TPW];
#pragma unroll
    for (int t = 0; t < TPW; ++t) {
      const f32x4 bv = *reinterpret_cast<const f32x4*>(sBias + (wid * TPW + t) * 16 + 4 * g);
#pragma unroll
      for (int i = 0; i < RT; ++i) acc[i][t] = bv;
    }
    if (real && wcol0 < q) {
#pragma unroll
      for (int s2 = 0; s2 < KS; ++s2) {
#pragma unroll
        for (int i = 0; i < RT; ++i) {
          const bf16x8 af = *reinterpret_cast<const bf16x8*>(st + (i * KS + s2) * 1024 + offA);
#pragma unroll
          for (int t = 0; t < TPW; ++t) acc[i][t] = __builtin_amdgcn_mfma_f32_16x16x32_bf16(bfr[t][s2], af, acc[i][t], 0, 0, 0);
        }
      }
    }
#pragma unroll
    for (int i = 0; i < RT; ++i) {
      const int ml = 16 * i + fr;
      const bool rok = real && ml < L;
      bf16_t* crow = a.e + (size_t)(row0 + ml) * a.lde;
      float pd = 0.f;
      uint2 pk[TPW];
#pragma unroll
      for (int t = 0; t < TPW; ++t) {
        bf16x4 o;
#pragma unroll
        for (int r = 0; r < 4; ++r) {
          const float th = 1.f - 2.f * __builtin_amdgcn_rcpf(__expf(2.f * acc[i][t][r]) + 1.f);
          o[r] = (bf16_t)th;
          pd = fmaf((float)o[r], w2r[t][r], pd);
        }
        pk[t] = __builtin_bit_cast(uint2, o);
      }
      const auto s0 = __builtin_amdgcn_permlane16_swap(pk[0].x, pk[1].x, false, false);
      const auto s1 = __builtin_amdgcn_permlane16_swap(pk[0].y, pk[1].y, false, false);
      const int col = wcol0 + (g & 1) * 16 + (g >> 1) * 8;
      uint4* dst = (rok && col + 8 <= q) ? reinterpret_cast<uint4*>(crow + col) : dump_g;
      *dst = make_uint4(s0[0], s1[0], s0[1], s1[1]);
      pd += __shfl_xor(pd, 16, 64);
      pd += __shfl_xor(pd, 32, 64);
      if (g == 0) sPart[((k & 1) * NW + wid) * 32 + ml] = pd;
    }
  };

#pragma unroll 1
  for (int k = 0; k < nsteps + 2; ++k) {
    if (k >= 2) asm volatile("s_waitcnt vmcnt(%0)" ::"n"(Cfg::STEADY) : "memory");
    else wait_vmcnt_le(k == 0 ? (NS - 3) * PW : PW + (Cfg::S + 2));
    __builtin_amdgcn_s_barrier();
    issue_stage(k + NS - 2);
    if (wid < NW / 2) {
      phase_gemm(k);
      phase_out(k);
      phase_alpha(k);
    } else {
      phase_out(k);
      phase_alpha(k);
      phase_gemm(k);
    }
  }
}

struct PoolFusedBwdArgs {
  const bf16_t* x; int ldx;
  const bf16_t* e; int lde;
  const float* alpha;
  const float* g; int ldg;
  const float* w2;
  const bf16_t* w1t; int ldw1t;
  bf16_t* dpre; int ldp;
  bf16_t* dx; int lddx;
  float* partial;
  const int32_t* nz;
  int n, L, N, q;
  int dx_far_unwritten;
};

template <int KS, int KS2>
struct PoolFusedBwdCfg {
  static constexpr int NW = 8, TPW = 4, RT = 2, R = 32;
  static constexpr int EPIECES = RT * KS2, GPIECES = 2, PIECES = EPIECES + GPIECES;
  static constexpr int PW = (PIECES + NW - 1) / NW, STAGE = PIECES * 1024, NS = 5;
  static constexpr int LOADS = 5;
  static constexpr int OPS = PW + LOADS + 2 + RT * 2;
  static constexpr int STEADY = 2 * OPS - PW;
  static constexpr int DUMP = NS * STAGE;
  static constexpr int PARTA = DUMP + NW * 1024;
  static constexpr int ALPHA = PARTA + 2 * NW * 32 * 4;
  static constexpr int W2 = ALPHA + 4 * 32 * 4;
  static constexpr int ACCW = W2 + 2 * 256 * 4;
  static constexpr int LIST = ACCW + 512 * 16 * 4;
  static_assert(STEADY <= 62, "vmcnt is a 6-bit counter");
};

template <int KS, int KS2>
__global__ __launch_bounds__(512) void pool_fused_bwd_kernel(PoolFusedBwdArgs a, int reach) {
  using Cfg = PoolFusedBwdCfg<KS, KS2>;
  constexpr int NW = Cfg::NW, TPW = Cfg::TPW, RT = Cfg::RT, NS = Cfg::NS, PW = Cfg::PW, STAGE = Cfg::STAGE, EPIECES = Cfg::EPIECES;
  extern __shared__ __attribute__((aligned(16))) char smem[];
  const uint32_t lds0 = (uint32_t)(size_t)(__attribute__((address_space(3))) char*)smem;
  const int tid = threadIdx.x, lane = tid & 63;
  const int wid = __builtin_amdgcn_readfirstlane(tid >> 6);
  const int fr = lane & 15, g = lane >> 4;
  const int prow = lane >> 2, c8 = ((lane & 3) ^ swzP(prow)) * 8;
  const int L = a.L, N = a.N, q = a.q, M = a.n * a.L, qc = q >> 3;
  float* sPartA = reinterpret_cast<float*>(smem + Cfg::PARTA);
  float* sAlpha = reinterpret_cast<float*>(smem + Cfg::ALPHA);
  float* sW2 = reinterpret_cast<float*>(smem + Cfg::W2);
  float* sRedW = sW2 + 256;
  int* sList = reinterpret_cast<int*>(smem + Cfg::LIST);

  const int G = gridDim.x, b0 = blockIdx.x;
  int nsteps = b0 < a.n ? (a.n - b0 + G - 1) / G : 0;
  if (a.nz != nullptr) {
    __shared__ int sCnt[NW + 1];
    const int cand = nsteps;
    const int run = pool_balanced_walk<NW>(a.nz, a.n, G, b0, sList, sCnt, wid, lane);
    for (int c = wid; c < cand; c += NW) {
      const int sq = b0 + c * G;
      if (a.nz[sq] != 0) continue;
      bool near = false;
      for (int t = max(0, sq - reach) + lane; t <= min(a.n - 1, sq + reach); t += 64) near |= a.nz[t] != 0;
      near = __ballot(near) != 0ull;
      const size_t r0 = (size_t)sq * L;
      const int xc = N >> 3;
      if (near || !a.dx_far_unwritten)
        for (int u = lane; u < L * xc; u += 64) {
          const int row = u / xc, ch = u - row * xc;
          *reinterpret_cast<uint4*>(a.dx + (r0 + row) * a.lddx + ch * 8) = make_uint4(0, 0, 0, 0);
        }
      if (near)
        for (int u = lane; u < L * qc; u += 64) {
          const int row = u / qc, ch = u - row * qc;
          *reinterpret_cast<uint4*>(a.dpre + (r0 + row) * a.ldp + ch * 8) = make_uint4(0, 0, 0, 0);
        }
    }
    nsteps = run;
  } else {
    for (int c = tid; c < nsteps; c += 512) sList[c] = b0 + c * G;
  }
  for (int c = tid; c < 256; c += 512) {
    sW2[c] = c < q ? a.w2[c] : 0.f;
    sRedW[c] = 0.f;
  }
  const int wcol0 = wid * TPW * 16;
  bf16x8 bfr[TPW][KS2];
#pragma unroll
  for (int t = 0; t < TPW; ++t) {
    const bf16_t* brow = a.w1t + (size_t)min(wcol0 + t * 16 + fr, N - 1) * a.ldw1t + 8 * g;
#pragma unroll
    for (int s2 = 0; s2 < KS2; ++s2) bfr[t][s2] = *reinterpret_cast<const bf16x8*>(brow + 32 * s2);
  }
  __builtin_amdgcn_s_waitcnt(0x0F70);
  __syncthreads();
  float* prow_out = a.partial + (size_t)blockIdx.x * (q + 1);
  if (nsteps == 0) {
    for (int c = tid; c <= q; c += 512) prow_out[c] = 0.f;
    return;
  }

  const uint32_t dump_lds = lds0 + Cfg::DUMP + wid * 1024;
  uint4* dump_g = g_nt_dump + wid * 64 + lane;
  auto issue_stage = [&](int kk) {
    const uint32_t slot = lds0 + (kk % NS) * STAGE;
    const bool real = kk < nsteps;
    const int sq = real ? sList[kk] : 0;
    const int row0 = sq * L;
#pragma unroll
    for (int u = 0; u < PW; ++u) {
      const int p = wid + NW * u;
      if (real && p < EPIECES) {
        const int i = p / KS2, s2 = p - i * KS2;
        const bf16_t* rp = a.e + (size_t)min(row0 + 16 * i + prow, M - 1) * a.lde + c8;
        dma16(rp + min(32 * s2, q - 8 - c8), slot + p * 1024);
      } else if (real && p < EPIECES + Cfg::GPIECES) {
        const int j = p - EPIECES;
        dma16(a.g + (size_t)sq * a.ldg + min(256 * j + 4 * lane, N - 4), slot + p * 1024);
      } else {
        dma16(a.e + c8, dump_lds);
      }
    }
  };
  const int ks0 = wid, ks1 = wid + NW;
  auto load_seq = [&](int kk, bf16x8 (&xf)[RT][2], float& al) {
    const int row0 = sList[kk < nsteps ? kk : 0] * L;
#pragma unroll
    for (int i = 0; i < RT; ++i) {
      const bf16_t* rp = a.x + (size_t)min(row0 + 16 * i + fr, M - 1) * a.ldx;
      xf[i][0] = *reinterpret_cast<const bf16x8*>(rp + min(32 * ks0 + 8 * g, N - 8));
      xf[i][1] = *reinterpret_cast<const bf16x8*>(rp + min(32 * ks1 + 8 * g, N - 8));
    }
    const int rowa = sList[(kk >= 1 && kk - 1 < nsteps) ? kk - 1 : 0] * L;
    al = a.alpha[min(rowa + (lane & 31), M - 1)];
  };
  auto g_frag = [&](const float* grow, int ks, bf16x8& hi, bf16x8& lo) {
    const int k0 = 32 * ks + 8 * g;
    const bool ok = ks < KS && k0 < N;
    const f32x4 v0 = *reinterpret_cast<const f32x4*>(grow + min(k0, N - 8));
    const f32x4 v1 = *reinterpret_cast<const f32x4*>(grow + min(k0, N - 8) + 4);
#pragma unroll
    for (int e2 = 0; e2 < 8; ++e2) {
      const float v = ok ? (e2 < 4 ? v0[e2] : v1[e2 - 4]) : 0.f;
      const bf16_t h = (bf16_t)v;
      hi[e2] = h;
      lo[e2] = (bf16_t)(v - (float)h);
    }
  };
  auto sum32 = [&](float v) {
    v += __builtin_bit_cast(float, __builtin_amdgcn_update_dpp(0, __builtin_bit_cast(int, v), 0x128, 0xf, 0xf, false));
    v += __builtin_bit_cast(float, __builtin_amdgcn_update_dpp(0, __builtin_bit_cast(int, v), 0x124, 0xf, 0xf, false));
    v += __builtin_bit_cast(float, __builtin_amdgcn_update_dpp(0, __builtin_bit_cast(int, v), 0x122, 0xf, 0xf, false));
    v += __builtin_bit_cast(float, __builtin_amdgcn_update_dpp(0, __builtin_bit_cast(int, v), 0x121, 0xf, 0xf, false));
    return v + __shfl_xor(v, 16, 64);
  };
  const int offA = fr * 64 + ((g ^ swzP(fr)) << 4);
  const uint32_t inv_qc = (uint32_t)((0x100000000ull + (uint32_t)qc - 1) / (uint32_t)qc);
  int brow[2], bcc[2];
#pragma unroll
  for (int j = 0; j < 2; ++j) {
    const uint32_t u = (uint32_t)(tid + 512 * j);
    uint32_t r = __umulhi(u, inv_qc);
    if (r * (uint32_t)qc > u) --r;
    brow[j] = (int)r;
    bcc[j] = (int)(u - r * (uint32_t)qc);
  }

  bf16x8 xf[RT][2];
  float al_nb, al_cur = 0.f;
  float* myacc = reinterpret_cast<float*>(smem + Cfg::ACCW) + tid * 8;
#pragma unroll
  for (int j = 0; j < 2; ++j) {
    *reinterpret_cast<f32x4*>(myacc + j * 4096) = (f32x4){0.f, 0.f, 0.f, 0.f};
    *reinterpret_cast<f32x4*>(myacc + j * 4096 + 4) = (f32x4){0.f, 0.f, 0.f, 0.f};
  }
  float accb = 0.f;

#pragma unroll 1
  for (int kk = 0; kk < 2; ++kk) issue_stage(kk);
  load_seq(0, xf, al_nb);

#pragma unroll 1
  for (int k = 0; k < nsteps + 2; ++k) {
    if (k >= 2) asm volatile("s_waitcnt vmcnt(%0)" ::"n"(Cfg::STEADY) : "memory");
    else wait_vmcnt_le(k == 0 ? PW + Cfg::LOADS : Cfg::OPS + Cfg::LOADS);
    __builtin_amdgcn_s_barrier();
    issue_stage(k + 2);
    auto phase_a = [&]()     {
      const bool real = k < nsteps;
      const float* grow = reinterpret_cast<const float*>(smem + (k % NS) * STAGE + EPIECES * 1024);
      f32x4 da[RT];
#pragma unroll
      for (int i = 0; i < RT; ++i) da[i] = (f32x4){0.f, 0.f, 0.f, 0.f};
      if (real) {
#pragma unroll
        for (int j = 0; j < 2; ++j) {
          bf16x8 hi, lo;
          g_frag(grow, j == 0 ? ks0 : ks1, hi, lo);
#pragma unroll
          for (int i = 0; i < RT; ++i) {
            da[i] = __builtin_amdgcn_mfma_f32_16x16x32_bf16(hi, xf[i][j], da[i], 0, 0, 0);
            da[i] = __builtin_amdgcn_mfma_f32_16x16x32_bf16(lo, xf[i][j], da[i], 0, 0, 0);
          }
        }
      }
      if (g == 0) {
#pragma unroll
        for (int i = 0; i < RT; ++i) sPartA[((k & 1) * NW + wid) * 32 + 16 * i + fr] = da[i][0];
      }
      al_cur = al_nb;
      load_seq(k + 1, xf, al_nb);
    };
    auto phase_b = [&]()     {
      const int kp = k - 1;
      const bool real = kp >= 0 && kp < nsteps;
      const int row0 = real ? sList[kp] * L : 0;
      const bool in = (lane & 31) < L;
      const float alv = in ? al_cur : 0.f;
      const float* part = sPartA + ((kp & 1) * NW) * 32 + (lane & 31);
      float dA = 0.f;
#pragma unroll
      for (int w = 0; w < NW; ++w) dA += part[w * 32];
      dA = in ? dA : 0.f;
      const float tsum = sum32(alv * dA);
      const float ds = alv * (dA - tsum);
      if (wid == 0 && lane < 32) sAlpha[(kp & 3) * 32 + lane] = alv;
      if (real) accb += sum32(ds);
      char* st = smem + ((kp + NS) % NS) * STAGE;
#pragma unroll
      for (int j = 0; j < 2; ++j) {
        const int row = brow[j], cc = bcc[j];
        const bool valid = real && row < L;
        const int rc = min(row, L - 1);
        const float dsr = __shfl(ds, rc, 64);
        const int eoff = ((rc >> 4) * KS2 + (cc >> 2)) * 1024 + (rc & 15) * 64 + (((cc & 3) ^ swzP(rc & 15)) << 4);
        const bf16x8 ev = *reinterpret_cast<const bf16x8*>(st + eoff);
        const f32x4 wa = *reinterpret_cast<const f32x4*>(sW2 + cc * 8), wb = *reinterpret_cast<const f32x4*>(sW2 + cc * 8 + 4);
        bf16x8 o;
        f32x4 a0 = *reinterpret_cast<const f32x4*>(myacc + j * 4096), a1 = *reinterpret_cast<const f32x4*>(myacc + j * 4096 + 4);
#pragma unroll
// ... 13 lines not shown
    };
    auto phase_c = [&]()     {
      const int kc = k - 2;
      const bool real = kc >= 0 && kc < nsteps;
      const int row0 = real ? sList[kc] * L : 0;
      const char* st = smem + ((kc + NS) % NS) * STAGE;
      const float* grow = reinterpret_cast<const float*>(st + EPIECES * 1024);
#pragma unroll
      for (int i = 0; i < RT; ++i) {
        f32x4 acc[TPW];
#pragma unroll
        for (int t = 0; t < TPW; ++t) acc[t] = (f32x4){0.f, 0.f, 0.f, 0.f};
        if (real && wcol0 < N) {
#pragma unroll
          for (int s2 = 0; s2 < KS2; ++s2) {
            const bf16x8 af = *reinterpret_cast<const bf16x8*>(st + (i * KS2 + s2) * 1024 + offA);
#pragma unroll
            for (int t = 0; t < TPW; ++t) acc[t] = __builtin_amdgcn_mfma_f32_16x16x32_bf16(bfr[t][s2], af, acc[t], 0, 0, 0);
          }
        }
        const int ml = 16 * i + fr;
        const bool rok = real && ml < L;
        const float al = sAlpha[((kc + 4) & 3) * 32 + ml];
        bf16_t* crow = a.dx + (size_t)(row0 + ml) * a.lddx;
#pragma unroll
        for (int t = 0; t < TPW; t += 2) {
          uint2 pk[2];
#pragma unroll
          for (int h = 0; h < 2; ++h) {
            const int lc = wcol0 + (t + h) * 16 + 4 * g;
            const f32x4 gq = *reinterpret_cast<const f32x4*>(grow + lc);
            const f32x4 v = acc[t + h];
            const bf16x4 o = {(bf16_t)(v[0] + al * gq[0]), (bf16_t)(v[1] + al * gq[1]), (bf16_t)(v[2] + al * gq[2]), (bf16_t)(v[3] + al * gq[3])};
            pk[h] = __builtin_bit_cast(uint2, o);
          }
          const auto s0 = __builtin_amdgcn_permlane16_swap(pk[0].x, pk[1].x, false, false);
          const auto s1 = __builtin_amdgcn_permlane16_swap(pk[0].y, pk[1].y, false, false);
          const int col = wcol0 + (t + (g & 1)) * 16 + (g >> 1) * 8;
          uint4* dst = (rok && col + 8 <= N) ? reinterpret_cast<uint4*>(crow + col) : dump_g;
          *dst = make_uint4(s0[0], s1[0], s0[1], s1[1]);
        }
      }
    };
    if (wid < NW / 2) {
      phase_a();
      phase_b();
      phase_c();
    } else {
      phase_c();
      phase_a();
      phase_b();
    }
  }
#pragma unroll
  for (int j = 0; j < 2; ++j)
#pragma unroll
    for (int e2 = 0; e2 < 8; ++e2) atomicAdd(sRedW + bcc[j] * 8 + e2, myacc[j * 4096 + e2]);
  __syncthreads();
  for (int c = tid; c < q; c += 512) prow_out[c] = sRedW[c];
  if (tid == 0) prow_out[q] = accb;
}

template <int EPI, int NT16, bool PK, int WM>
int launch_nt_dma_w(const RowSrc& A, const void* B, int ldb, int M, int N, int K, const EpiArgs& ep, hipStream_t stream) {
  constexpr int DBM = 64 * WM, NP = DBM / 16 + NT16, STAGE = NP * 1024, NS = dma_ring_stages(STAGE, WM);
  constexpr size_t ring = (size_t)NS * STAGE, epi = (size_t)32 * (NT16 * 16 + 4) * sizeof(float);
  constexpr size_t epk = PK ? (size_t)128 * (NT16 * 16 + 8) * sizeof(bf16_t) : 0;
  constexpr size_t gtile = EPI == EPI_POOLBWD && PK ? (size_t)((12 * NT16 * 16 * 4 + 1023) / 1024) * 1024 + 1024
                                                    : ((EPI == EPI_SCATTER || EPI == EPI_STORE) ? 2048 : 1024);
  constexpr size_t smem0 = ring > epi ? ring : epi, smem1 = smem0 > epk ? smem0 : epk, smem = smem1 + gtile;
  auto kern = gemm_nt_dma_kernel<EPI, NT16, PK, WM>;
  NR_CHECK_HIP(hipFuncSetAttribute(reinterpret_cast<const void*>(kern), hipFuncAttributeMaxDynamicSharedMemorySize, (int)smem));
  const int tilesM = (M + DBM - 1) / DBM, nchunks = (N + NT16 * 16 - 1) / (NT16 * 16);
  int grid = ((tilesM + 7) / 8) * 8 * nchunks;
  EpiArgs epl = ep;
  epl.tail_cus = 0;
  if constexpr (EPI == EPI_SCATTER && !PK && WM == 4) {
    if (ep.row_count != nullptr && nchunks == 1) {
      static int cus = 0;
      if (cus == 0) {
        int dev = 0, c = 0;
        NR_CHECK_HIP(hipGetDevice(&dev));
        NR_CHECK_HIP(hipDeviceGetAttribute(&c, hipDeviceAttributeMultiprocessorCount, dev));
        cus = c >= 8 ? c : 256;
      }
      epl.tail_cus = cus;
      grid = nr_scatter_tail_grid(M, cus);
    }
  }
  hipLaunchKernelGGL(kern, dim3(grid), dim3(128 * WM), smem, stream, (const bf16_t*)A.base, A.ld, (const bf16_t*)B, ldb, M, N, K, epl, nchunks);
  NR_CHECK_LAUNCH();
  return NR_OK;
}

template <int EPI, int NT16, bool PK>
int launch_nt_dma_p(const RowSrc& A, const void* B, int ldb, int M, int N, int K, const EpiArgs& ep, hipStream_t stream) {
  constexpr bool fits2 = 3 * (8 + NT16) * 1024 <= 78 * 1024;
  if (fits2 && (N <= 2 * NT16 * 16 || K <= 224)) return launch_nt_dma_w<EPI, NT16, PK, 2>(A, B, ldb, M, N, K, ep, stream);
  return launch_nt_dma_w<EPI, NT16, PK, 4>(A, B, ldb, M, N, K, ep, stream);
}

template <int EPI, int NT16>
int launch_nt_dma_t(const RowSrc& A, const void* B, int ldb, int M, int N, int K, const EpiArgs& ep, hipStream_t stream) {
  if (EPI != EPI_SCATTER && ep.out_dtype == NR_BF16) return launch_nt_dma_p<EPI, NT16, true>(A, B, ldb, M, N, K, ep, stream);
  return launch_nt_dma_p<EPI, NT16, false>(A, B, ldb, M, N, K, ep, stream);
}

template <int NT16>
int launch_nt_dma_e(const RowSrc& A, const void* B, int ldb, int M, int N, int K, int epi, const EpiArgs& ep, hipStream_t s) {
  switch (epi) {
    case EPI_STORE: return launch_nt_dma_t<EPI_STORE, NT16>(A, B, ldb, M, N, K, ep, s);
    case EPI_STORE_TANH: return launch_nt_dma_t<EPI_STORE_TANH, NT16>(A, B, ldb, M, N, K, ep, s);
// ... 804 lines not shown
}

int nr_launch_rows_materialize(int dtype, const RowSrc& A, void* out, int ldo, int M, int K, hipStream_t stream, const int32_t* needed,
                               int margin, int L, const int32_t* keep_all) {
  const int ch = nr_chunk(dtype);
  NR_CHECK_ARG((A.kind == ROWS_GATHER || A.kind == ROWS_IM2COL3) && K % ch == 0 && ldo % ch == 0 && ldo >= K, "rows_materialize: bad arguments");
  if (needed != nullptr && A.kind == ROWS_GATHER && L > 0 && M % L == 0 && keep_all != nullptr) {
    NrProfScope ps(stream, "rows_materialize_needed[%s,Mmax=%d,K=%d]", dtype == NR_BF16 ? "bf16" : "f32", M, K);
    const int n = M / L;
    if (dtype == NR_BF16)
      hipLaunchKernelGGL(gather_title_kernel<bf16_t>, dim3(n), dim3(256), 0, stream, A, (bf16_t*)out, ldo, M, K, L, needed, n, margin, keep_all);
    else
      hipLaunchKernelGGL(gather_title_kernel<float>, dim3(n), dim3(256), 0, stream, A, (float*)out, ldo, M, K, L, needed, n, margin, keep_all);
    NR_CHECK_LAUNCH();
    return NR_OK;
  }
  if (needed != nullptr && A.kind == ROWS_IM2COL3 && K == 3 * A.ld && M % A.Tlen == 0) {
    NrProfScope ps(stream, "rows_materialize_needed[%s,Mmax=%d,K=%d]", dtype == NR_BF16 ? "bf16" : "f32", M, K);
    const int n = M / A.Tlen;
    if (dtype == NR_BF16)
      hipLaunchKernelGGL(im2col3_title_kernel<bf16_t>, dim3(n), dim3(256), 0, stream, A, (bf16_t*)out, ldo, M, needed, n, margin);
    else
      hipLaunchKernelGGL(im2col3_title_kernel<float>, dim3(n), dim3(256), 0, stream, A, (float*)out, ldo, M, needed, n, margin);
    NR_CHECK_LAUNCH();
    return NR_OK;
  }
  NrProfScope ps(stream, "rows_materialize[%s,M=%d,K=%d]", dtype == NR_BF16 ? "bf16" : "f32", M, K);
  const size_t total = (size_t)M * (K / ch);
  size_t grid = (total + 255) / 256;
  if (grid > 256 * 32) grid = 256 * 32;
  if (A.kind == ROWS_IM2COL3) {
    NR_CHECK_ARG(K == 3 * A.ld && A.ld % ch == 0, "rows_materialize: im2col rows are [M, 3*Dp]");
    size_t g3 = ((size_t)M * (A.ld / ch) + 255) / 256;
    if (g3 > 256 * 32) g3 = 256 * 32;
    if (dtype == NR_BF16)
      hipLaunchKernelGGL(im2col3_materialize_kernel<bf16_t>, dim3((unsigned)g3), dim3(256), 0, stream, A, (bf16_t*)out, ldo, M);
    else
      hipLaunchKernelGGL(im2col3_materialize_kernel<float>, dim3((unsigned)g3), dim3(256), 0, stream, A, (float*)out, ldo, M);
  } else if (dtype == NR_BF16)
    hipLaunchKernelGGL((rows_materialize_kernel<bf16_t, ROWS_GATHER>), dim3((unsigned)grid), dim3(256), 0, stream, A, (bf16_t*)out, ldo, M, K);
  else
    hipLaunchKernelGGL((rows_materialize_kernel<float, ROWS_GATHER>), dim3((unsigned)grid), dim3(256), 0, stream, A, (float*)out, ldo, M, K);
  NR_CHECK_LAUNCH();
  return NR_OK;
}

int nr_pool_fused_fwd_ok(int dtype, int n, int L, int N, int q, int ldw1) {
  return !nr_opt(NR_OPT_NO_POOL_FUSED) && dtype == NR_BF16 && L >= 24 && L <= 32 && N > 384 && N <= 416 && N % 8 == 0 && q >= 8 && q <= 256 &&
         q % 8 == 0 && ldw1 >= 416 && (long)n * L >= 4096;
}

int nr_launch_pool_fused_fwd(const void* x, int ldx, const void* w1, int ldw1, const float* b1, const float* w2, const float* b2,
                             const float* mask, void* e, int lde, float* alpha, float* out, int ld_out, int n, int L, int N, int q,
                             const int32_t* needed, hipStream_t stream) {
  constexpr int KS = 13;
  using Cfg = PoolFusedCfg<KS>;
  NR_CHECK_ARG(nr_pool_fused_fwd_ok(NR_BF16, n, L, N, q, ldw1) && ldx >= N && ldx % 8 == 0 && lde >= q && lde % 8 == 0 &&
                   ((((uintptr_t)x) | ((uintptr_t)w1) | ((uintptr_t)e)) & 15) == 0 && mask == nullptr,
               "pool_fused_fwd: shape / alignment not eligible (and no mask on this path)");
  static int cus = 0;
  if (cus == 0) {
    int dev = 0, c = 0;
    NR_CHECK_HIP(hipGetDevice(&dev));
    NR_CHECK_HIP(hipDeviceGetAttribute(&c, hipDeviceAttributeMultiprocessorCount, dev));
    cus = c >= 8 ? c : 256;
  }
  const int grid = n < cus ? n : cus;
  const int max_steps = (n + grid - 1) / grid;
  const size_t smem = (size_t)Cfg::LIST + (size_t)(max_steps + 8) * sizeof(int);
  NR_CHECK_ARG(smem <= 160 * 1024, "pool_fused_fwd: %d sequences per workgroup do not fit the LDS list", max_steps);
  PoolFusedArgs a;
  a.x = (const bf16_t*)x; a.ldx = ldx; a.w1 = (const bf16_t*)w1; a.ldw1 = ldw1; a.b1 = b1; a.w2 = w2; a.b2 = b2;
  a.e = (bf16_t*)e; a.lde = lde; a.alpha = alpha; a.out = out; a.ld_out = ld_out; a.needed = needed; a.n = n; a.L = L; a.N = N; a.q = q;
  auto kern = pool_fused_fwd_kernel<KS>;
  NR_CHECK_HIP(hipFuncSetAttribute(reinterpret_cast<const void*>(kern), hipFuncAttributeMaxDynamicSharedMemorySize, (int)smem));
  NrProfScope ps(stream, needed ? "pool_fused_fwd_needed[bf16,n=%d,L=%d,N=%d,q=%d]" : "pool_fused_fwd[bf16,n=%d,L=%d,N=%d,q=%d]", n, L, N, q);
  hipLaunchKernelGGL(kern, dim3(grid), dim3(512), smem, stream, a, max_steps);
  NR_CHECK_LAUNCH();
  return NR_OK;
}

int nr_pool_fused_bwd_ok(int dtype, int n, int L, int N, int q, int ldw1t) {
  return !nr_opt(NR_OPT_NO_POOL_FUSED) && dtype == NR_BF16 && L >= 24 && L <= 32 && N > 384 && N <= 416 && N % 8 == 0 && q > 192 && q <= 224 &&
         q % 8 == 0 && ldw1t >= 224 && (long)n * L >= 4096;
}

int nr_launch_pool_fused_bwd(const void* x, int ldx, const void* e, int lde, const float* alpha, const float* g, int ldg, const float* w2,
                             const void* w1t, int ldw1t, void* dpre, int ldp, void* dx, int lddx, float* partial, int partial_rows,
                             const int32_t* nz, int n, int L, int N, int q, hipStream_t stream, int* grid_out, int dx_far_unwritten) {
  constexpr int KS = 13, KS2 = 7;
  using Cfg = PoolFusedBwdCfg<KS, KS2>;
  NR_CHECK_ARG(nr_pool_fused_bwd_ok(NR_BF16, n, L, N, q, ldw1t) && ldx >= N && ldx % 8 == 0 && lde >= q && lde % 8 == 0 && ldp >= q && ldp % 8 == 0 &&
                   lddx >= N && lddx % 8 == 0 && ldg >= N && ldg % 4 == 0 &&
                   ((((uintptr_t)x) | ((uintptr_t)e) | ((uintptr_t)w1t) | ((uintptr_t)dpre) | ((uintptr_t)dx) | ((uintptr_t)g)) & 15) == 0,
               "pool_fused_bwd: shape / alignment not eligible");
  static int cus = 0;
  if (cus == 0) {
    int dev = 0, c = 0;
    NR_CHECK_HIP(hipGetDevice(&dev));
    NR_CHECK_HIP(hipDeviceGetAttribute(&c, hipDeviceAttributeMultiprocessorCount, dev));
    cus = c >= 8 ? c : 256;
  }
  int grid = n < cus ? n : cus;
  if (grid > partial_rows) grid = partial_rows;
  const int max_steps = (n + grid - 1) / grid;
  const size_t smem = (size_t)Cfg::LIST + (size_t)(max_steps + 8) * sizeof(int);
  NR_CHECK_ARG(smem <= 160 * 1024, "pool_fused_bwd: %d sequences per workgroup do not fit the LDS list", max_steps);
  PoolFusedBwdArgs a;
  a.x = (const bf16_t*)x; a.ldx = ldx; a.e = (const bf16_t*)e; a.lde = lde; a.alpha = alpha; a.g = g; a.ldg = ldg; a.w2 = w2;
  a.w1t = (const bf16_t*)w1t; a.ldw1t = ldw1t; a.dpre = (bf16_t*)dpre; a.ldp = ldp; a.dx = (bf16_t*)dx; a.lddx = lddx; a.partial = partial;
  a.nz = nz; a.n = n; a.L = L; a.N = N; a.q = q; a.dx_far_unwritten = (nz != nullptr && dx_far_unwritten) ? 1 : 0;
  auto kern = pool_fused_bwd_kernel<KS, KS2>;
  NR_CHECK_HIP(hipFuncSetAttribute(reinterpret_cast<const void*>(kern), hipFuncAttributeMaxDynamicSharedMemorySize, (int)smem));
  NrProfScope ps(stream, "pool_fused_bwd[bf16,n=%d,L=%d,N=%d,q=%d]", n, L, N, q);
  hipLaunchKernelGGL(kern, dim3(grid), dim3(512), smem, stream, a, 32 / L + 2);
  NR_CHECK_LAUNCH();
  *grid_out = grid;
  return NR_OK;
}

int nr_launch_gather_live_rows(int dtype, const RowSrc& A, void* out, int ldo, int Mmax, int K, const int32_t* count, const int32_t* rows,
                               const int32_t* ids, hipStream_t stream, int32_t* hist, int V) {
  const int ch = nr_chunk(dtype);
  NR_CHECK_ARG(A.kind == ROWS_GATHER && K % ch == 0 && ldo % ch == 0 && ldo >= K && A.ld >= K && count && rows && ids && out,
               "gather_live_rows: bad arguments");
  NrProfScope ps(stream, "rows_materialize_live[%s,Mmax=%d,K=%d]", dtype == NR_BF16 ? "bf16" : "f32", Mmax, K);
  const size_t total = (size_t)Mmax * (K / ch);
  size_t grid = (total + 256 * 4 - 1) / (256 * 4);
  if (grid > 256 * 16) grid = 256 * 16;
  if (grid < 1) grid = 1;
  if (dtype == NR_BF16)
    hipLaunchKernelGGL(gather_live_rows_kernel<bf16_t>, dim3((unsigned)grid), dim3(256), 0, stream, A, (bf16_t*)out, ldo, K, count, rows, ids, hist, V);
  else
    hipLaunchKernelGGL(gather_live_rows_kernel<float>, dim3((unsigned)grid), dim3(256), 0, stream, A, (float*)out, ldo, K, count, rows, ids, hist, V);
  NR_CHECK_LAUNCH();
  return NR_OK;
}

int nr_launch_gemm_nt(int dtype, const RowSrc& A, const void* B, int ldb, int M, int N, int K, int epi, const EpiArgs& ep,
                      hipStream_t stream) {
  const int ch = nr_chunk(dtype);
  NR_CHECK_ARG(M > 0 && N > 0 && K > 0, "gemm_nt: empty problem M=%d N=%d K=%d", M, N, K);
  NR_CHECK_ARG(K % ch == 0 && ldb % ch == 0 && A.ld % ch == 0, "gemm_nt: K=%d ldb=%d lda=%d must be multiples of %d", K, ldb, A.ld, ch);
  NR_CHECK_ARG(((uintptr_t)A.base & 15) == 0 && ((uintptr_t)B & 15) == 0, "gemm_nt: operands must be 16-byte aligned");
  if (epi != EPI_SCATTER) NR_CHECK_ARG(ep.ldc % 4 == 0 && ((uintptr_t)ep.C & 15) == 0, "gemm_nt: output ld %d / alignment", ep.ldc);
  if (epi == EPI_STORE && ep.act_tanh) epi = EPI_STORE_TANH;
  constexpr int DMA_MIN_K = 192;
  const int kr32 = (K + 31) / 32 * 32;
  const bool dense_bf16 = dtype == NR_BF16 && A.kind == ROWS_DENSE && A.drop.thresh == 0 && ep.rows_out == nullptr;
  if (dense_bf16 && K >= DMA_MIN_K && ldb >= kr32 && (A.ld >= K || A.gap > 0)) {
    EpiArgs epg = ep;
    epg.a_gap = A.gap;
    const EpiArgs& ep = epg;
    const bool tile_skip = (epi == EPI_STORE || epi == EPI_STORE_TANH) && ep.seq_nz != nullptr && ep.row_count == nullptr;
    if (nr_opt(NR_OPT_NT_WREG) && A.gap == 0 && ep.out_dtype == NR_BF16 && N % 8 == 0 && ep.ldc % 8 == 0 && M >= 64 && ldb >= kr32 &&
        (ep.row_count == nullptr || (((uintptr_t)ep.row_idx & 15) == 0 && M % 4 == 0))) {
      const bool flags = ep.seq_nz != nullptr && ep.row_count == nullptr && ep.L >= 16;
      const char* lbl = ep.row_count ? "gemm_nt_wreg_live[bf16,epi=%d,Mmax=%d,N=%d,K=%d]"
                                     : (ep.seq_nz ? "gemm_nt_wreg_needed[bf16,epi=%d,Mmax=%d,N=%d,K=%d]" : "gemm_nt_wreg[bf16,epi=%d,M=%d,N=%d,K=%d]");
      if (epi == EPI_STORE && !tile_skip && K > 288 && K <= 320 && N >= 320) {
        NrProfScope ps(stream, lbl, epi, M, N, K);
        if (ep.row_count && ep.a_dense) return launch_nt_wreg_m<EPI_STORE, 5, 10, 2, WREG_COMPACT_DENSE, true>(A, B, ldb, M, N, K, ep, stream);
        return ep.row_count ? launch_nt_wreg_m<EPI_STORE, 5, 10, 2, WREG_COMPACT, true>(A, B, ldb, M, N, K, ep, stream)
                            : launch_nt_wreg_m<EPI_STORE, 5, 10, 2, WREG_DENSE, true>(A, B, ldb, M, N, K, ep, stream);
// ... 214 lines not shown
  __shared__ int base;
  const int tid = threadIdx.x, lane = tid & 63, wid = tid >> 6;
  const int i = blockIdx.x * 256 + tid;
  bool keep = false;
  if (i < n) {
    bool skip = tmask[i] == 0;
    for (int j = max(0, i - margin); skip && j <= min(n - 1, i + margin); ++j) skip = title_nz[j] == 0;
    keep = !skip;
  }
  const uint64_t bal = __ballot(keep);
  if (lane == 0) wave_cnt[wid] = __popcll(bal);
  __syncthreads();
  if (tid == 0) base = atomicAdd(count, wave_cnt[0] + wave_cnt[1] + wave_cnt[2] + wave_cnt[3]);
  __syncthreads();
  if (keep) {
    int pos = base + __popcll(bal & ((1ull << lane) - 1ull));
    for (int w = 0; w < wid; ++w) pos += wave_cnt[w];
    list[pos] = i;
  }
}
}
namespace {
__global__ __launch_bounds__(256) void needed_list_kernel(const int32_t* __restrict__ flags, int n, int32_t* __restrict__ count,
                                                          int32_t* __restrict__ list) {
  __shared__ int wave_cnt[4];
  __shared__ int base;
  const int tid = threadIdx.x, lane = tid & 63, wid = tid >> 6;
  const int i = blockIdx.x * 256 + tid;
  const bool keep = i < n && flags[i] != 0;
  const uint64_t bal = __ballot(keep);
  if (lane == 0) wave_cnt[wid] = __popcll(bal);
  __syncthreads();
  if (tid == 0) base = atomicAdd(count, wave_cnt[0] + wave_cnt[1] + wave_cnt[2] + wave_cnt[3]);
  __syncthreads();
  if (keep) {
    int pos = base + __popcll(bal & ((1ull << lane) - 1ull));
    for (int w = 0; w < wid; ++w) pos += wave_cnt[w];
    list[pos] = i;
  }
}
__global__ __launch_bounds__(256) void zero_unneeded_kernel(const int32_t* __restrict__ flags, uint4* __restrict__ y, int chunks16, int n,
                                                            int reach) {
  const int seq = blockIdx.x;
  if (flags[seq] != 0) return;
  if (reach >= 0) {
    bool near = false;
    for (int t = max(0, seq - reach) + (int)threadIdx.x; t <= min(n - 1, seq + reach); t += 256) near |= flags[t] != 0;
    if (!__syncthreads_or(near)) return;
  }
  uint4* p = y + (size_t)seq * chunks16;
  for (int c = threadIdx.x; c < chunks16; c += 256) p[c] = make_uint4(0, 0, 0, 0);
}
}
int nr_launch_needed_list(const int32_t* flags, int n, int32_t* out, void* y, size_t seq_bytes, hipStream_t stream, int reach, bool zeroed) {
  NR_CHECK_ARG(flags != nullptr && out != nullptr && y != nullptr && seq_bytes % 16 == 0 && (((uintptr_t)y) & 15) == 0, "needed_list: bad arguments");
  if (!zeroed) NR_CHECK_HIP(hipMemsetAsync(out, 0, 4 * sizeof(int32_t), stream));
  NrProfScope ps(stream, "needed_list[n=%d]", n);
  hipLaunchKernelGGL(needed_list_kernel, dim3((n + 255) / 256), dim3(256), 0, stream, flags, n, out, out + 4);
  hipLaunchKernelGGL(zero_unneeded_kernel, dim3(n), dim3(256), 0, stream, flags, reinterpret_cast<uint4*>(y), (int)(seq_bytes / 16), n, reach);
  NR_CHECK_LAUNCH();
  return NR_OK;
}

int nr_launch_seq_list(const int32_t* title_nz, const uint32_t* tmask, int n, int L, int32_t* out, hipStream_t stream, int reach, bool zeroed) {
  if (!zeroed) NR_CHECK_HIP(hipMemsetAsync(out, 0, 4 * sizeof(int32_t), stream));
  hipLaunchKernelGGL(seq_list_kernel, dim3((n + 255) / 256), dim3(256), 0, stream, title_nz, tmask, n, reach >= 0 ? reach : 32 / L + 2, out,
                     out + 4);
  NR_CHECK_LAUNCH();
  return NR_OK;
}

namespace {
__global__ __launch_bounds__(256) void zero_tail_rows_kernel(uint4* __restrict__ buf, int chunks, const int32_t* __restrict__ count, int Mmax,
                                                             int32_t* __restrict__ za, int na, int32_t* __restrict__ zb, int nb) {
  const int t = blockIdx.x * 256 + threadIdx.x, stride = gridDim.x * 256;
  for (int i = t; i < na; i += stride) za[i] = 0;
  for (int i = t; i < nb; i += stride) zb[i] = 0;
  if (blockIdx.x != 0) return;
  const int n = *count, end = min(Mmax, (n + 31) / 32 * 32);
  for (int u = threadIdx.x; u < (end - n) * chunks; u += 256) buf[(size_t)n * chunks + u] = make_uint4(0, 0, 0, 0);
}
}
int nr_launch_zero_tail_rows(void* buf, int ld, const int32_t* count, int Mmax, hipStream_t stream, int32_t* za, int na, int32_t* zb, int nb) {
  NR_CHECK_ARG(buf != nullptr && count != nullptr && ld % 8 == 0 && (((uintptr_t)buf) & 15) == 0, "zero_tail_rows: bad arguments");
  if (za == nullptr) na = 0;
  if (zb == nullptr) nb = 0;
  const int most = na > nb ? na : nb, grid = most > 4096 ? 16 : 1;
  hipLaunchKernelGGL(zero_tail_rows_kernel, dim3(grid), dim3(256), 0, stream, (uint4*)buf, ld / 8, count, Mmax, za, na, zb, nb);
  NR_CHECK_LAUNCH();
  return NR_OK;
}

int nr_launch_live_slabs(int32_t* ws, int n, int L, hipStream_t stream) {
  const int M = n * L, nslab = M / 32;
  NR_CHECK_ARG(ws != nullptr && M % 32 == 0, "live_slabs: bad arguments");
  int32_t* list = ws + n + 4;
  if (nslab >= 4 && nslab <= 128 * 1024) {
    unsigned char* flags = reinterpret_cast<unsigned char*>(list + nslab - (nslab + 3) / 4);
    hipLaunchKernelGGL(slab_flags_kernel, dim3((nslab + 255) / 256), dim3(256), 0, stream, ws, n, L, nslab, flags);
    hipLaunchKernelGGL(slab_list_kernel, dim3(1), dim3(1024), (size_t)((nslab + 15) / 16) * 16, stream, flags, nslab, ws + n, list);
    NR_CHECK_LAUNCH();
    return NR_OK;
  }
  const int in_lds = n <= 128 * 1024 ? 1 : 0;
  hipLaunchKernelGGL(live_slabs_kernel, dim3(1), dim3(1024), in_lds ? (size_t)((n + 15) / 16) * 16 : 0, stream, ws, n, L, nslab, ws + n,
                     list, in_lds);
  NR_CHECK_LAUNCH();
  return NR_OK;
}

int nr_launch_gemm_tn_slabs(const void* dC, int ldc, const void* X, int ldx, float* dW, int ldw, float* db, int M, int N, int K,
                            int Nstore, int Kstore, const int32_t* slab_list, const int32_t* slab_count, hipStream_t stream, int xgap,
// ... 36 lines not shown
```

newsrecommendation_amd/model/NRMS.py:

```python
import torch
from torch import nn

from .. import ops
from .model_utils import AttentionPooling, MultiHeadSelfAttention


def _cd(args):
    return getattr(args, "compute_dtype", "fp32")


class NewsEncoder(nn.Module):

    def __init__(self, args, embedding_matrix):
        super().__init__()
        self.embedding_matrix = embedding_matrix
        self.drop_rate = args.drop_rate
        self.dim_per_head = args.news_dim // args.num_attention_heads
        assert args.news_dim == args.num_attention_heads * self.dim_per_head
        self.multi_head_self_attn = MultiHeadSelfAttention(args.word_embedding_dim, args.num_attention_heads,
                                                           self.dim_per_head, self.dim_per_head, compute_dtype=_cd(args))
        self.attn = AttentionPooling(args.news_dim, args.news_query_vector_dim, compute_dtype=_cd(args))

    def forward(self, x, mask=None, needed=None):
        p = self.drop_rate if self.training else 0.0
        needed = ops.needed_flags(needed)
        far = needed is not None and ops.pool_contracts_slabs(x.shape[0], x.shape[1], self.attn.att_fc1.in_features,
                                                              self.attn.att_fc1.out_features, ops.dtype_code(self.attn.compute_dtype))
        y = self.multi_head_self_attn.forward_gather(x, self.embedding_matrix.weight, mask=mask, p_in=p, p_out=p, needed=needed,
                                                     far_unwritten=far)
        return self.attn(y, mask, needed=needed, lazy_dx=far and getattr(y, "_nr_takes_lazy_dy", False))


class UserEncoder(nn.Module):

    def __init__(self, args):
        super().__init__()
        self.args = args
        self.dim_per_head = args.news_dim // args.num_attention_heads
        assert args.news_dim == args.num_attention_heads * self.dim_per_head
        self.multi_head_self_attn = MultiHeadSelfAttention(args.news_dim, args.num_attention_heads, self.dim_per_head,
                                                           self.dim_per_head, compute_dtype=_cd(args))
        self.attn = AttentionPooling(args.news_dim, args.user_query_vector_dim, compute_dtype=_cd(args))
        self.pad_doc = nn.Parameter(torch.empty(1, args.news_dim).uniform_(-1, 1)).type(torch.FloatTensor)

    def forward(self, news_vecs, log_mask=None):
        code = ops.dtype_code(_cd(self.args))
        if self.args.user_log_mask:
            x = news_vecs if news_vecs.dtype == ops.torch_dtype(code) else ops.to_compute(news_vecs.float(), code)
            y = self.multi_head_self_attn(x, mask=log_mask)
            return self.attn(y, log_mask)
        x = ops.pad_blend(news_vecs, log_mask, self.pad_doc, code)
        y = self.multi_head_self_attn(x)
        return self.attn(y)


    @torch.no_grad()
    def forward_indexed(self, news_table, history_idx, log_mask):
        if not self.args.user_log_mask or ops.dtype_code(_cd(self.args)) != ops.NR_BF16 or history_idx.shape[1] > 64:
            code = ops.dtype_code(_cd(self.args)) if self.args.user_log_mask else ops.NR_F32
            return self.forward(ops.embed_gather(news_table, history_idx, code), log_mask)
        y = self.multi_head_self_attn.forward_gather(history_idx, news_table, mask=log_mask)
        return self.attn(y, log_mask)


class Model(torch.nn.Module):

    def __init__(self, args, embedding_matrix, *unused, **kwargs):
        super().__init__()
        self.args = args
        pretrained_word_embedding = torch.from_numpy(embedding_matrix).float()
        word_embedding = nn.Embedding.from_pretrained(pretrained_word_embedding, freeze=args.freeze_embedding, padding_idx=0)
        self.news_encoder = NewsEncoder(args, word_embedding)
        self.user_encoder = UserEncoder(args)
        self.loss_fn = nn.CrossEntropyLoss()

    def forward(self, history, history_mask, candidate, label):
        a = self.args
        B = candidate.shape[0]
        C = 1 + a.npratio
        cand = candidate.reshape(-1, a.num_words_title)
        hist = history.reshape(-1, a.num_words_title)
        compact = getattr(a, "compact_history", False)
        if compact:
# ... 19 lines not shown
```

newsrecommendation_amd/model/model_utils.py:

```python
import torch
from torch import nn

from .. import ops


class AttentionPooling(nn.Module):

    def __init__(self, emb_size, hidden_size, compute_dtype="fp32"):
        super().__init__()
        self.att_fc1 = nn.Linear(emb_size, hidden_size)
        self.att_fc2 = nn.Linear(hidden_size, 1)
        self.compute_dtype = compute_dtype

    def forward(self, x, attn_mask=None, needed=None, lazy_dx=False):
        code = ops.dtype_code(self.compute_dtype)
        if x.dtype != ops.torch_dtype(code):
            x = ops.to_compute(x.float(), code)
            lazy_dx = False
        return ops.additive_pool(x, self.att_fc1.weight, self.att_fc1.bias, self.att_fc2.weight, self.att_fc2.bias,
                                 code, mask=attn_mask, needed=needed, lazy_dx=lazy_dx)


class ScaledDotProductAttention(nn.Module):

    def __init__(self, d_k, compute_dtype="fp32"):
        super().__init__()
        self.d_k = d_k
        self.compute_dtype = compute_dtype

    def forward(self, Q, K, V, attn_mask=None):
        if Q.shape[-1] != self.d_k:
            raise RuntimeError(f"ScaledDotProductAttention(d_k={self.d_k}) got head dim {Q.shape[-1]}")
        return ops.sdpa(Q, K, V, ops.dtype_code(self.compute_dtype), mask=attn_mask)


class MultiHeadSelfAttention(nn.Module):

    def __init__(self, d_model, n_heads, d_k, d_v, compute_dtype="fp32"):
        super().__init__()
        if d_k != d_v:
            raise ValueError("d_k must equal d_v (as at every reference call site)")
        self.d_model, self.n_heads, self.d_k, self.d_v = d_model, n_heads, d_k, d_v
        self.W_Q = nn.Linear(d_model, d_k * n_heads)
        self.W_K = nn.Linear(d_model, d_k * n_heads)
        self.W_V = nn.Linear(d_model, d_v * n_heads)
        self.scaled_dot_product_attn = ScaledDotProductAttention(self.d_k, compute_dtype=compute_dtype)
        self.compute_dtype = compute_dtype
        self._initialize_weights()

    def _initialize_weights(self):
        for m in self.modules():
            if isinstance(m, nn.Linear):
                nn.init.xavier_uniform_(m.weight, gain=1)

    def _params(self):
        return (self.W_Q.weight, self.W_Q.bias, self.W_K.weight, self.W_K.bias, self.W_V.weight, self.W_V.bias)

    def forward(self, Q, K=None, V=None, mask=None, p_out=0.0):
        if (K is not None and K is not Q) or (V is not None and V is not Q):
            raise NotImplementedError("only self-attention (Q is K is V) exists in the reference and here")
        code = ops.dtype_code(self.compute_dtype)
        x = Q
        if x.dtype != ops.torch_dtype(code):
            x = ops.to_compute(x.float(), code)
        return ops.mhsa(x, *self._params(), heads=self.n_heads, code=code, mask=mask, p_out=p_out,
                        flat=getattr(self, "_nr_flat", None))

    def forward_gather(self, ids, table, mask=None, p_in=0.0, p_out=0.0, needed=None, far_unwritten=False):
        code = ops.dtype_code(self.compute_dtype)
        return ops.mhsa(None, *self._params(), heads=self.n_heads, code=code, mask=mask, ids=ids, table=table,
                        p_in=p_in, p_out=p_out, flat=getattr(self, "_nr_flat", None), needed=needed, far_unwritten=far_unwritten)
```

newsrecommendation_amd/ops.py:

```python
from __future__ import annotations

import ctypes as C
import os
import weakref
from typing import Optional

import torch
from torch.autograd import Function

from . import _lib
from ._lib import NR_BF16, NR_F32, NR_SRC_DENSE, NR_SRC_GATHER, check, ptr

_DTYPES = {"fp32": NR_F32, "f32": NR_F32, "float32": NR_F32, "bf16": NR_BF16, "bfloat16": NR_BF16}


def dtype_code(name) -> int:
    if isinstance(name, int):
        return name
    try:
        return _DTYPES[str(name).lower()]
    except KeyError:
        raise ValueError(f"compute dtype must be one of {sorted(_DTYPES)}, got {name!r}")


# ... 257 lines not shown
            w_p = pack(wcat, code)
            if w_p.shape[1] != tp.shape[1]:
                raise RuntimeError(f"projected table: operand leading dimensions differ ({w_p.shape[1]} vs {tp.shape[1]})")
            proj = gemm_nt(tp, w_p, bias=bcat.detach().float().contiguous())
            if id(table) not in self._c:
                weakref.finalize(table, self._c.pop, id(table), None)
            ent = (sig, proj, weakref.ref(table))
            self._c[id(table)] = ent
        return ent[1]


projected_tables = _ProjectedTables()


class MHSAFunction(Function):

    @staticmethod
    def forward(ctx, x, wq, bq, wk, bk, wv, bv, ids, mask, cfg):
        _need_gpu(x, wq, ids, mask)
        code, heads, gather = cfg["code"], cfg["heads"], ids is not None
        N, d_model = wq.shape
        d_head = N // heads
        ch = chunk(code)
        if gather:
            n, L = ids.shape
            src = cfg["table_packed"]
            ids = ids.contiguous()
        else:
            n, L, _ = x.shape
            src = x.contiguous()
            if src.dtype != torch_dtype(code):
                raise RuntimeError(f"dense MHSA input must be {torch_dtype(code)}, got {src.dtype}")
        ldx = src.shape[-1]
        flat = cfg.get("flat")
        if flat is not None:
            wcat, b_p = flat["w"], flat["b"]
        else:
            wcat = torch.cat([wq, wk, wv], dim=0)
            b_p = torch.cat([bq, bk, bv]).detach().float().contiguous()
        w_p = pack(wcat, code)
        mask_c = mask.contiguous().float() if mask is not None else None
        dev = wq.device
        y = _scratch(n, L, N, dtype=torch_dtype(code), device=dev)
        need_bwd = any(ctx.needs_input_grad[:7])
        keep_rows = gather and any(ctx.needs_input_grad[1:7])
        Kp = round_up(d_model, ch)
        x_rows = torch.empty(n * L, Kp, dtype=torch_dtype(code), device=dev) if keep_rows else None
        d = _lib.MhsaDesc(n=n, L=L, d_model=d_model, heads=heads, d_head=d_head, dtype=code,
                          src_kind=NR_SRC_GATHER if gather else NR_SRC_DENSE, x=ptr(src), ldx=ldx, ids=ptr(ids),
                          p_in=cfg["p_in"], seed_in=cfg["seed_in"], p_out=cfg["p_out"], seed_out=cfg["seed_out"],
                          mask=ptr(mask_c), w_qkv=ptr(w_p), ldw=w_p.shape[1], b_qkv=ptr(b_p),
                          x_rows=ptr(x_rows), ld_rows=Kp, seq_needed=ptr(cfg.get("needed")),
                          y_far_unwritten=int(bool(cfg.get("far_unwritten")) and cfg.get("needed") is not None),
                          table_rows=cfg["table_shape"][0] if gather else 0)
        row_ws = _ws(_lib.lib().nr_mhsa_workspace_bytes(C.byref(d)), dev) if keep_rows and code == _lib.NR_BF16 else None
        d.row_ws, d.row_ws_bytes = ptr(row_ws), (row_ws.numel() * 4 if row_ws is not None else 0)
        fused = bool(_lib.lib().nr_mhsa_fwd_fused(C.byref(d)))
        qkv = None if (fused and not need_bwd) else _scratch(n * L, 3 * N, dtype=torch_dtype(code), device=dev)
        check(_lib.lib().nr_mhsa_fwd(C.byref(d), ptr(qkv), ptr(y), _stream()), "nr_mhsa_fwd")
        cfg["compact_rows"] = bool(keep_rows and _lib.lib().nr_mhsa_compact_rows(C.byref(d)))
        ctx.cfg, ctx.dims = cfg, (n, L, N, d_model, heads, d_head, ldx, gather)
        ctx.row_ws = row_ws
        ctx.save_for_backward(src, ids, mask_c, w_p, b_p, wcat, qkv, x_rows)
        return y

    @staticmethod
    def backward(ctx, dy):
        seq = _enter_backward()
        src, ids, mask_c, w_p, b_p, wcat, qkv, x_rows = ctx.saved_tensors
        cfg = ctx.cfg
        n, L, N, d_model, heads, d_head, ldx, gather = ctx.dims
        code, dev = cfg["code"], dy.device
        dy = dy.contiguous()
        if dy.dtype != torch_dtype(code):
            dy = dy.to(torch_dtype(code))
        seq_nz, seq_nz_owner, dy_lazy = _take_flags(seq, dy, n)
        dqkv = _scratch(*qkv.shape, dtype=qkv.dtype, device=dev)
        bucket = cfg.get("flat")
        if bucket is not None:
            dw, db = bucket["gw"], bucket["gb"]
        else:
            flat = torch.zeros(3 * N * d_model + 3 * N, dtype=torch.float32, device=dev)
            dw, db = flat[:3 * N * d_model].view(3 * N, d_model), flat[3 * N * d_model:]
        need_x = ctx.needs_input_grad[0]
        dx = dtable = w_t = None
        row_ws = getattr(ctx, "row_ws", None)
        ws_ready = row_ws is not None
        d = _lib.MhsaDesc(n=n, L=L, d_model=d_model, heads=heads, d_head=d_head, dtype=code,
                          src_kind=NR_SRC_GATHER if gather else NR_SRC_DENSE, x=ptr(src), ldx=ldx, ids=ptr(ids),
                          p_in=cfg["p_in"], seed_in=cfg["seed_in"], p_out=cfg["p_out"], seed_out=cfg["seed_out"],
                          mask=ptr(mask_c), w_qkv=ptr(w_p), ldw=w_p.shape[1], b_qkv=ptr(b_p),
                          x_rows=ptr(x_rows), ld_rows=x_rows.shape[1] if x_rows is not None else 0,
                          table_rows=cfg["table_shape"][0] if gather else 0, seq_nz=seq_nz, row_ws_ready=int(ws_ready),
                          dy_far_unwritten=int(dy_lazy),
                          seq_needed=ptr(cfg.get("needed")))
        if need_x:
            w_t = pack(wcat, code, transpose=True)
            if gather:
                dtable = cfg.get("table_grad")
                if dtable is None:
                    dtable = torch.zeros(cfg["table_shape"], dtype=torch.float32, device=dev)
                if row_ws is None:
                    row_ws = _ws(_lib.lib().nr_mhsa_workspace_bytes(C.byref(d)), dev)
            else:
                dx = torch.empty(n, L, ldx, dtype=torch_dtype(code), device=dev)
        d.row_ws, d.row_ws_bytes = ptr(row_ws), (row_ws.numel() * 4 if row_ws is not None else 0)
        def run(phase):
            d.bwd_phase = phase
            check(_lib.lib().nr_mhsa_bwd(C.byref(d), ptr(qkv), ptr(dy), ptr(dqkv), ptr(w_t), w_t.shape[1] if w_t is not None else 0,
                                         ptr(dw), ptr(db), ptr(dx), ptr(dtable), _stream()), "nr_mhsa_bwd")
        ready = cfg.get("table_grad_ready") if (gather and cfg.get("table_grad") is not None and _det_scratch is None) else None
        if ready is not None:
            run(1)
            ready()
            run(2)
        else:
            run(0)
        gx = (None if cfg.get("table_grad") is not None else dtable) if gather else dx
        if bucket is not None:
            return (gx, None, None, None, None, None, None, None, None, None)
        return (gx, dw[:N], db[:N], dw[N:2 * N], db[N:2 * N], dw[2 * N:], db[2 * N:], None, None, None)


USE_PROJECTED_TABLE = True


def _mhsa_projected(table, params, flat, ids, mask, heads, code, p_out):
    wq, bq, wk, bk, wv, bv = params
    if flat is not None:
        wcat, bcat = flat["w"], flat["b"]
    else:
        wcat, bcat = torch.cat([wq, wk, wv], dim=0), torch.cat([bq, bk, bv])
    proj = projected_tables.get(table, params, wcat, bcat, code)
    n, L = ids.shape
    N, d_model = wq.shape
    mask_c = mask.contiguous().float() if mask is not None else None
    y = torch.empty(n, L, N, dtype=torch_dtype(code), device=ids.device)
    tp = table_cache.get(table, code)
    d = _lib.MhsaDesc(n=n, L=L, d_model=d_model, heads=heads, d_head=N // heads, dtype=code, src_kind=NR_SRC_GATHER, x=ptr(tp),
                      ldx=tp.shape[1], ids=ptr(ids), p_in=0.0, seed_in=0, p_out=p_out, seed_out=draw_seed() if p_out > 0 else 0,
                      mask=ptr(mask_c), w_qkv=ptr(proj), ldw=tp.shape[1], b_qkv=ptr(proj), proj_table=ptr(proj))
    check(_lib.lib().nr_mhsa_fwd(C.byref(d), None, ptr(y), _stream()), "nr_mhsa_fwd")
    return y


def needed_flags(needed):
    if needed is None:
        return None
    if getattr(needed, "_nr_flags01", False):
        return needed
    return (needed.reshape(-1) != 0).to(torch.int32).contiguous()


def pool_contracts_slabs(n: int, L: int, N: int, q: int, code: int) -> bool:
    d = _lib.PoolDesc(n=int(n), L=int(L), N=int(N), q=int(q), dtype=int(code))
    return bool(_lib.lib().nr_pool_contracts_slabs(C.byref(d)))


def mhsa(x, wq, bq, wk, bk, wv, bv, heads: int, code: int, mask=None, ids=None, table=None, p_in=0.0, p_out=0.0, flat=None,
         needed=None, far_unwritten=False):
    cfg = dict(code=code, heads=heads, p_in=float(p_in), p_out=float(p_out),
               seed_in=draw_seed() if p_in > 0 else 0, seed_out=draw_seed() if p_out > 0 else 0, needed=needed,
               far_unwritten=bool(far_unwritten))
    if flat is not None:
        cfg["flat"] = flat
    if ids is not None:
        if ids.dtype != torch.int32:
            ids = ids.to(torch.int32)
        if CHECK_INDICES:
            check_ids(ids, table.shape[0], "token id")
        N = wq.shape[0]
        if (not torch.is_grad_enabled() and p_in == 0 and code == NR_BF16 and ids.dim() == 2 and ids.shape[1] <= 64
                and (N // heads) % 4 == 0 and N % 8 == 0 and USE_PROJECTED_TABLE):
            return _mhsa_projected(table, (wq, bq, wk, bk, wv, bv), flat, ids.contiguous(), mask, heads, code, float(p_out))
        cfg["table_packed"] = table_cache.get(table, code)
        cfg["table_shape"] = tuple(table.shape)
        if table.requires_grad and torch.is_grad_enabled():
            cfg["table_grad"] = grad_target(table)
            cfg["table_grad_ready"] = getattr(table, "_nr_grad_ready", None)
        y = MHSAFunction.apply(table, wq, bq, wk, bk, wv, bv, ids, mask, cfg)
        y._nr_takes_lazy_dy = bool(cfg.get("compact_rows"))
        return y
    ch = chunk(code)
    if x.shape[-1] % ch:
        pad = ch - x.shape[-1] % ch
        cfg.pop("flat", None)
        x = torch.nn.functional.pad(x, (0, pad))
        wq, wk, wv = (torch.nn.functional.pad(w, (0, pad)) for w in (wq, wk, wv))
    return MHSAFunction.apply(x, wq, bq, wk, bk, wv, bv, None, mask, cfg)


class SDPAFunction(Function):

    @staticmethod
    def forward(ctx, qkv, mask, n, L, heads, d_head, code):
        _need_gpu(qkv, mask)
        N = heads * d_head
        mask_c = mask.contiguous().float() if mask is not None else None
        y = torch.empty(n * L, N, dtype=torch_dtype(code), device=qkv.device)
        check(_lib.lib().nr_sdpa_fwd(ptr(qkv), ptr(mask_c), ptr(y), n, L, heads, d_head, code, 0.0, 0, _stream()), "nr_sdpa_fwd")
        ctx.dims = (n, L, heads, d_head, code)
        ctx.save_for_backward(qkv, mask_c)
        return y

    @staticmethod
    def backward(ctx, dy):
        _enter_backward()
        qkv, mask_c = ctx.saved_tensors
        n, L, heads, d_head, code = ctx.dims
        dy = dy.contiguous()
        if dy.dtype != torch_dtype(code):
            dy = dy.to(torch_dtype(code))
        dqkv = torch.empty_like(qkv)
        check(_lib.lib().nr_sdpa_bwd(ptr(qkv), ptr(mask_c), ptr(dy), ptr(dqkv), n, L, heads, d_head, code, 0.0, 0, _stream()),
              "nr_sdpa_bwd")
        return dqkv, None, None, None, None, None, None


class LongSDPAFunction(Function):

    @staticmethod
    def forward(ctx, qkv, mask, n, L, heads, d_head, code):
        _need_gpu(qkv, mask)
        N = heads * d_head
        mask_c = mask.contiguous().float() if mask is not None else None
        y = torch.empty(n * L, N, dtype=torch_dtype(code), device=qkv.device)
        check(_lib.lib().nr_sdpa_long_fwd(ptr(qkv), ptr(mask_c), ptr(y), n, L, heads, d_head, code, 0.0, 0, _stream()),
              "nr_sdpa_long_fwd")
        ctx.dims = (n, L, heads, d_head, code)
        ctx.save_for_backward(qkv, mask_c)
        return y

    @staticmethod
    def backward(ctx, dy):
        _enter_backward()
        qkv, mask_c = ctx.saved_tensors
        n, L, heads, d_head, code = ctx.dims
        dy = dy.contiguous()
        if dy.dtype != torch_dtype(code):
            dy = dy.to(torch_dtype(code))
        dqkv = torch.empty_like(qkv)
        check(_lib.lib().nr_sdpa_long_bwd(ptr(qkv), ptr(mask_c), ptr(dy), ptr(dqkv), n, L, heads, d_head, code, 0.0, 0, _stream()),
              "nr_sdpa_long_bwd")
        return dqkv, None, None, None, None, None, None


def sdpa(Q, K, V, code: int, mask=None):
    _need_gpu(Q, K, V, mask)
    n, h, L, d = Q.shape
    if K.shape != Q.shape or V.shape != Q.shape:
        raise RuntimeError(f"sdpa: Q/K/V shapes differ: {tuple(Q.shape)}, {tuple(K.shape)}, {tuple(V.shape)} (d_k must equal d_v)")
    if mask is not None and mask.dim() == 3:
        if mask.stride(1) != 0 and not bool((mask == mask[:, :1]).all()):
            raise NotImplementedError("sdpa: per-head attention masks do not occur in the reference (the mask is the [n, L] key "
                                      "mask repeated over heads, src/model/model_utils.py:86-87) and are not supported")
        mask = mask[:, 0]
    td = torch_dtype(code)
    qkv = torch.stack([t.to(td).permute(0, 2, 1, 3) for t in (Q, K, V)], dim=2).reshape(n * L, 3 * h * d)
    y = (LongSDPAFunction if L > 64 else SDPAFunction).apply(qkv, mask, n, L, h, d, code)
    return y.view(n, L, h, d).permute(0, 2, 1, 3)


class PoolFunction(Function):

    @staticmethod
    def forward(ctx, x, w1, b1, w2, b2, mask, code, needed=None, lazy_dx=False):
        _need_gpu(x, w1, mask)
        n, L, N = x.shape
        q = w1.shape[0]
        x = x.contiguous()
        if x.dtype != torch_dtype(code):
            raise RuntimeError(f"pool input must be {torch_dtype(code)}, got {x.dtype}")
        dev = x.device
        w1_p = pack(w1, code)
        b1_c, w2_c, b2_c = (t.detach().float().contiguous() for t in (b1, w2.reshape(-1), b2))
        mask_c = mask.contiguous().float() if mask is not None else None
        e = torch.empty(n * L, q, dtype=torch_dtype(code), device=dev)
        alpha = torch.empty(n * L, dtype=torch.float32, device=dev)
        out = torch.empty(n, N, dtype=torch.float32, device=dev)
        d = _lib.PoolDesc(n=n, L=L, N=N, q=q, dtype=code, x=ptr(x), mask=ptr(mask_c), w1=ptr(w1_p), ldw1=w1_p.shape[1],
                          b1=ptr(b1_c), w2=ptr(w2_c), b2=ptr(b2_c), seq_needed=ptr(needed))
        check(_lib.lib().nr_additive_pool_fwd(C.byref(d), ptr(e), ptr(alpha), ptr(out), N, _stream()), "nr_additive_pool_fwd")
        ctx.code, ctx.dims = code, (n, L, N, q)
        ctx.needed = needed
        ctx.lazy_dx = bool(lazy_dx)
        ctx.targets = tuple(grad_target(p) for p in (w1, b1, w2, b2))
        ctx.save_for_backward(x, mask_c, w1_p, b1_c, w2_c, b2_c, e, alpha, w1)
        return out

    @staticmethod
    def backward(ctx, g):
        seq = _enter_backward()
        x, mask_c, w1_p, b1_c, w2_c, b2_c, e, alpha, w1 = ctx.saved_tensors
        n, L, N, q = ctx.dims
        code, dev = ctx.code, g.device
        g = g.contiguous().float()
        w1_t = pack(w1, code, transpose=True) if ctx.needs_input_grad[0] else None
        dpre = torch.empty_like(e)
        direct = all(t is not None for t in ctx.targets)
        if direct:
            dw1, db1, dw2, db2 = ctx.targets
        else:
            flat = torch.zeros(q * N + 2 * q + 4, dtype=torch.float32, device=dev)
            dw1, db1, dw2, db2 = flat[:q * N].view(q, N), flat[q * N:q * N + q], flat[q * N + q:q * N + 2 * q], flat[q * N + 2 * q:q * N + 2 * q + 1]
        dx = torch.empty_like(x) if ctx.needs_input_grad[0] else None
        d = _lib.PoolDesc(n=n, L=L, N=N, q=q, dtype=code, x=ptr(x), mask=ptr(mask_c), w1=ptr(w1_p), ldw1=w1_p.shape[1],
                          b1=ptr(b1_c), w2=ptr(w2_c), b2=ptr(b2_c), seq_needed=ptr(ctx.needed), dx_far_unwritten=int(ctx.lazy_dx))
        partial = _ws(_lib.lib().nr_pool_workspace_bytes(C.byref(d)), dev)
        d.partial_bytes = partial.numel() * 4
        check(_lib.lib().nr_additive_pool_bwd(C.byref(d), ptr(e), ptr(alpha), ptr(g), N, ptr(w1_t),
                                              w1_t.shape[1] if w1_t is not None else 0, ptr(dpre), ptr(partial), ptr(dw1),
                                              ptr(db1), ptr(dw2), ptr(db2), ptr(dx), _stream()), "nr_additive_pool_bwd")
        flags_ptr = _lib.lib().nr_pool_seq_flags(C.byref(d), ptr(partial))
        _offer_flags(seq, dx, n, flags_ptr, partial, lazy=ctx.lazy_dx and bool(flags_ptr))
        if direct:
            return dx, None, None, None, None, None, None, None, None
        return dx, dw1, db1, dw2.view(1, q), db2, None, None, None, None


def additive_pool(x, w1, b1, w2, b2, code: int, mask=None, needed=None, lazy_dx=False):
    return PoolFunction.apply(x, w1, b1, w2, b2, mask, code, needed, bool(lazy_dx) and x.requires_grad)


_grad_out = {}


def _take_grad_out(x):
    if not _grad_out or not x.is_cuda or x.dtype != torch.float32 or not x.is_contiguous():
        return None
    return _grad_out.pop((x.data_ptr(), x.numel()), None)


class SplitRowsFunction(Function):
    @staticmethod
    def forward(ctx, x, n_a):
        ctx.n_a, ctx.arena = int(n_a), None
        a, b = x[:n_a], x[n_a:]
        _grad_out.clear()
        if (ctx.needs_input_grad[0] and x.is_cuda and x.dtype == torch.float32 and x.is_contiguous() and x.dim() == 2
                and 0 < n_a < x.shape[0]):
            ctx.arena = torch.empty_like(x)
            _grad_out[(a.data_ptr(), a.numel())] = ctx.arena[:n_a]
            _grad_out[(b.data_ptr(), b.numel())] = ctx.arena[n_a:]
        return a, b

    @staticmethod
    def backward(ctx, ga, gb):
        arena, n_a = ctx.arena, ctx.n_a
        if (arena is not None and ga is not None and gb is not None and ga.dtype == gb.dtype == torch.float32 and ga.is_contiguous()
                and gb.is_contiguous() and ga.data_ptr() == arena.data_ptr() and gb.data_ptr() == arena[n_a:].data_ptr()
                and ga.numel() == arena[:n_a].numel() and gb.numel() == arena[n_a:].numel()):
            return arena, None
        return torch.cat([ga, gb], dim=0), None


def split_rows(x, n_a: int):
    return SplitRowsFunction.apply(x, n_a)


class BlendFunction(Function):

    @staticmethod
    def forward(ctx, x, mask, pad, code):
        _need_gpu(x, mask, pad)
        n, L, N = x.shape
        x = x.contiguous().float()
        mask_c = mask.contiguous().float() if mask is not None else None
        pad_c = pad.detach().reshape(-1).float().contiguous() if pad is not None else None
        out = torch.empty(n, L, N, dtype=torch_dtype(code), device=x.device)
        check(_lib.lib().nr_pad_blend_fwd(ptr(x), ptr(mask_c), ptr(pad_c), ptr(out), n, L, N, code, _stream()), "nr_pad_blend_fwd")
        ctx.code, ctx.dims, ctx.pad_shape = code, (n, L, N), (tuple(pad.shape) if pad is not None else None)
        ctx.pad_target = grad_target(pad)
        ctx.dx_out = _take_grad_out(x)
        ctx.save_for_backward(mask_c)
# ... 1673 lines not shown
```

Before: 173,900 impressions/s.

## Defer zero-fill of skipped sequences into fused pool kernels' pipelined stores

The MHSA forward no longer zero-fills the output rows of skipped sequences. The fused additive-pool forward now does this fill instead, interleaving one 16-byte zero store per pipeline step into its steady-state loop. The pool backward replaces its upfront per-sequence zeroing of dx/dpre with the same interleaved fill list, and gains a three-level laziness flag that can skip dx zeroing entirely. It also drops the shared-memory atomic reduction for dw2 partials in favour of a direct sum over the accumulator buffer. The aim is to hide memset traffic and a separate fill pass behind GEMM work. In exchange the vmcnt accounting is tighter, there is extra LDS list space, and correctness now depends on the ordering between producer and consumer.

```diff
diff --git a/include/nrhip.h b/include/nrhip.h
--- a/include/nrhip.h
+++ b/include/nrhip.h
@@ -74,6 +74,7 @@
   int bwd_phase;
   int y_far_unwritten;
   int dy_far_unwritten;
+  int y_zeros_deferred;
 } nr_mhsa_desc;
 
 int nr_mhsa_fwd_fused(const nr_mhsa_desc* d);
@@ -132,7 +133,9 @@
   size_t partial_bytes;
   const int32_t* seq_needed;
   int dx_far_unwritten;
+  int x_zero_near;
 } nr_pool_desc;
+int nr_pool_fills_x_zeros(const nr_pool_desc* d);
 int nr_pool_contracts_slabs(const nr_pool_desc* d);
 size_t nr_pool_workspace_bytes(const nr_pool_desc* d);
 const int32_t* nr_pool_seq_flags(const nr_pool_desc* d, const float* partial);
diff --git a/newsrecommendation_amd/_lib.py b/newsrecommendation_amd/_lib.py
--- a/newsrecommendation_amd/_lib.py
+++ b/newsrecommendation_amd/_lib.py
@@ -24,7 +24,7 @@
                 ("mask", C.c_void_p), ("w_qkv", C.c_void_p), ("ldw", C.c_int), ("b_qkv", C.c_void_p),
                 ("x_rows", C.c_void_p), ("ld_rows", C.c_int), ("row_ws", C.c_void_p), ("row_ws_bytes", C.c_size_t),
                 ("table_rows", C.c_int), ("proj_table", C.c_void_p), ("seq_needed", C.c_void_p), ("seq_nz", C.c_void_p), ("row_ws_ready", C.c_int), ("bwd_phase", C.c_int),
-                ("y_far_unwritten", C.c_int), ("dy_far_unwritten", C.c_int)]
+                ("y_far_unwritten", C.c_int), ("dy_far_unwritten", C.c_int), ("y_zeros_deferred", C.c_int)]
 
 
 class ConvDesc(C.Structure):
@@ -212,7 +212,8 @@
 class PoolDesc(C.Structure):
     _fields_ = [("n", C.c_int), ("L", C.c_int), ("N", C.c_int), ("q", C.c_int), ("dtype", C.c_int), ("x", C.c_void_p),
                 ("mask", C.c_void_p), ("w1", C.c_void_p), ("ldw1", C.c_int), ("b1", C.c_void_p), ("w2", C.c_void_p),
-                ("b2", C.c_void_p), ("partial_bytes", C.c_size_t), ("seq_needed", C.c_void_p), ("dx_far_unwritten", C.c_int)]
+                ("b2", C.c_void_p), ("partial_bytes", C.c_size_t), ("seq_needed", C.c_void_p), ("dx_far_unwritten", C.c_int),
+                ("x_zero_near", C.c_int)]
 
 
 class LinearDesc(C.Structure):
@@ -242,6 +243,7 @@
     "nr_conv_table_workspace_bytes": [C.POINTER(ConvDesc)],
     "nr_pool_workspace_bytes": [C.POINTER(PoolDesc)],
     "nr_pool_contracts_slabs": [C.POINTER(PoolDesc)],
+    "nr_pool_fills_x_zeros": [C.POINTER(PoolDesc)],
     "nr_pool_seq_flags": [C.POINTER(PoolDesc), _vp],
     "nr_linear_workspace_bytes": [C.POINTER(LinearDesc)],
     "nr_sdpa_fwd": [_vp, _vp, _vp, _i, _i, _i, _i, _i, _f, _u32, _vp],
diff --git a/newsrecommendation_amd/csrc/nr_api.hip b/newsrecommendation_amd/csrc/nr_api.hip
--- a/newsrecommendation_amd/csrc/nr_api.hip
+++ b/newsrecommendation_amd/csrc/nr_api.hip
@@ -499,6 +499,12 @@
 int nr_pool_contracts_slabs(const nr_pool_desc* d) {
   return (d != nullptr && d->n > 0 && d->L >= 1 && d->q >= 1 && dtype_ok(d->dtype) && pool_has_flags(d)) ? 1 : 0;
 }
+static bool pool_fwd_fused(const nr_pool_desc* d) {
+  return nr_pool_fused_fwd_ok(d->dtype, d->n, d->L, d->N, d->q, d->ldw1) && d->N % 8 == 0 && d->mask == nullptr;
+}
+int nr_pool_fills_x_zeros(const nr_pool_desc* d) {
+  return (d != nullptr && d->n > 0 && d->L >= 1 && d->N >= 1 && d->q >= 1 && dtype_ok(d->dtype) && pool_fwd_fused(d)) ? 1 : 0;
+}
 size_t nr_pool_workspace_bytes(const nr_pool_desc* d) {
   return (d == nullptr || d->n < 0 || d->L < 1 || d->q < 1) ? 0 : pool_ws_elems(d->n, d->L, d->q, d->N, d->dtype) * sizeof(float);
 }
@@ -656,6 +662,8 @@
   if (rc) return rc;
   if (d->n == 0) return NR_OK;
   NR_CHECK_ARG(y != nullptr, "mhsa_fwd: null output");
+  NR_CHECK_ARG(!d->y_zeros_deferred || (d->seq_needed != nullptr && d->y_far_unwritten),
+               "mhsa_fwd: y_zeros_deferred needs seq_needed and y_far_unwritten (the consumer fills the near rows only)");
   hipStream_t s = (hipStream_t)stream;
   NR_DEVICE_GUARD(stream, y);
   const int N = d->heads * d->d_head, M = P.M, Kp = P.Kp;
@@ -709,7 +717,8 @@
   if (P.needed_list && tmask != nullptr && aligned(16, y)) {
     int32_t* lw = ws + W.seq;
     if ((rc = nr_launch_needed_list(d->seq_needed, d->n, lw, y, (size_t)d->L * N * nr_elt_size(d->dtype), s,
-                                    d->y_far_unwritten ? 32 / d->L + 2 : -1, true)))
+                                    d->y_far_unwritten ? 32 / d->L + 2 : -1, true,
+                                    !d->y_zeros_deferred)))
       return rc;
     fwd_list = lw;
   }
@@ -983,12 +992,16 @@
   if (rc) return rc;
   if (d->n == 0) return NR_OK;
   NR_CHECK_ARG(e && alpha && out && ld_out >= d->N, "additive_pool_fwd: null output / ld_out");
+  const bool fused = pool_fwd_fused(d) && ((((uintptr_t)d->x) | ((uintptr_t)d->w1) | ((uintptr_t)e)) & 15) == 0;
+  NR_CHECK_ARG(!d->x_zero_near || d->seq_needed != nullptr, "additive_pool_fwd: x_zero_near needs the seq_needed flags");
+  NR_CHECK_ARG(!d->x_zero_near || fused,
+               "additive_pool_fwd: x_zero_near is only honoured by the fused forward (nr_pool_fills_x_zeros() says 0, or x / w1 / e are not "
+               "16-byte aligned)");
   NR_DEVICE_GUARD(stream, out);
   hipStream_t s = (hipStream_t)stream;
-  if (nr_pool_fused_fwd_ok(d->dtype, d->n, d->L, d->N, d->q, d->ldw1) && ((((uintptr_t)d->x) | ((uintptr_t)d->w1) | ((uintptr_t)e)) & 15) == 0 &&
-      d->N % 8 == 0 && d->mask == nullptr)
+  if (fused)
     return nr_launch_pool_fused_fwd(d->x, d->N, d->w1, d->ldw1, d->b1, d->w2, d->b2, d->mask, e, d->q, alpha, out, ld_out, d->n, d->L, d->N, d->q,
-                                    d->seq_needed, s);
+                                    d->seq_needed, s, d->x_zero_near);
   RowSrc A = dense_rows(d->x, d->N, d->N);
   EpiArgs ep = store_epi(e, d->q, d->dtype, d->b1, 1);
   ep.seq_nz = d->seq_needed; ep.L = d->L;
diff --git a/newsrecommendation_amd/csrc/nr_gemm.h b/newsrecommendation_amd/csrc/nr_gemm.h
--- a/newsrecommendation_amd/csrc/nr_gemm.h
+++ b/newsrecommendation_amd/csrc/nr_gemm.h
@@ -65,7 +65,7 @@
 int nr_launch_row_flags_f32(const float* g, int ld, int N, int n, int32_t* nz, hipStream_t stream);
 int nr_launch_live_slabs(int32_t* ws, int n, int L, hipStream_t stream);
 int nr_launch_needed_list(const int32_t* flags, int n, int32_t* out, void* y, size_t seq_bytes, hipStream_t stream, int reach = -1,
-                          bool zeroed = false);
+                          bool zeroed = false, bool fill = true);
 int nr_launch_seq_list(const int32_t* title_nz, const uint32_t* tmask, int n, int L, int32_t* out, hipStream_t stream, int reach = -1,
                        bool zeroed = false);
 int nr_launch_zero_tail_rows(void* buf, int ld, const int32_t* count, int Mmax, hipStream_t stream, int32_t* za = nullptr, int na = 0,
@@ -78,7 +78,7 @@
 int nr_pool_fused_fwd_ok(int dtype, int n, int L, int N, int q, int ldw1);
 int nr_launch_pool_fused_fwd(const void* x, int ldx, const void* w1, int ldw1, const float* b1, const float* w2, const float* b2,
                              const float* mask, void* e, int lde, float* alpha, float* out, int ld_out, int n, int L, int N, int q,
-                             const int32_t* needed, hipStream_t stream);
+                             const int32_t* needed, hipStream_t stream, int x_zero_near = 0);
 int nr_launch_gemm_tn_counted(const void* dC, int ldc, const void* X, int ldx, float* dW, int ldw, int Mmax, int N, int K, int Nstore,
                               int Kstore, const int32_t* row_count, hipStream_t stream, float* scratch = nullptr, size_t scratch_floats = 0);
 int nr_pool_fused_bwd_ok(int dtype, int n, int L, int N, int q, int ldw1t);
diff --git a/newsrecommendation_amd/csrc/nr_gemm.hip b/newsrecommendation_amd/csrc/nr_gemm.hip
--- a/newsrecommendation_amd/csrc/nr_gemm.hip
+++ b/newsrecommendation_amd/csrc/nr_gemm.hip
@@ -1689,6 +1689,57 @@
   return b0 < total ? (total - b0 + G - 1) / G : 0;
 }
 
+struct PoolFillCfg {
+  static constexpr int Z = 1;
+};
+
+template <int NW>
+__device__ __forceinline__ int pool_fill_cap(int n, int G) { return ((n + G - 1) / G + NW - 1) / NW; }
+
+template <int NW, class KindOf>
+__device__ __forceinline__ int pool_fill_list(const int32_t* __restrict__ flags, int n, int G, int b0, int cand, int reach, int* myFill, int wid,
+                                              int lane, KindOf kind_of) {
+  int nfill = 0;
+  for (int c0 = 0; c0 < cand; c0 += NW * 64) {
+    const int c = c0 + wid + NW * lane;
+    const int sq = b0 + c * G;
+    int kind = 0;
+    if (c < cand && flags[sq] == 0) {
+      bool near = false;
+      for (int t = max(0, sq - reach); t <= min(n - 1, sq + reach); ++t) near |= flags[t] != 0;
+      kind = kind_of(near);
+    }
+    const uint64_t bal = __ballot(kind != 0);
+    if (kind != 0) myFill[nfill + __popcll(bal & ((1ull << lane) - 1ull))] = sq * 4 + kind;
+    nfill += __popcll(bal);
+  }
+  return nfill;
+}
+
+struct PoolFillDst {
+  bf16_t* a; int lda, ca;
+  bf16_t* b; int ldb, cb;
+  int L;
+};
+
+__device__ __forceinline__ void pool_fill_store(const int* myFill, int nfill, int& ent, int& pc, const PoolFillDst& f, int lane, uint4* dump_g) {
+  uint4* dst = dump_g;
+  if (ent < nfill) {
+    const int en = __builtin_amdgcn_readfirstlane(myFill[ent]);
+    const int na = (en & 1) ? (f.L * f.ca + 63) >> 6 : 0, nb = (en & 2) ? (f.L * f.cb + 63) >> 6 : 0;
+    const bool isa = pc < na;
+    const int cr = isa ? f.ca : f.cb, ld = isa ? f.lda : f.ldb;
+    const int u = ((isa ? pc : pc - na) << 6) + lane;
+    const int row = (int)((uint32_t)u / (uint32_t)cr), ch = u - row * cr;
+    if (row < f.L) dst = reinterpret_cast<uint4*>((isa ? f.a : f.b) + ((size_t)(en >> 2) * f.L + row) * ld + ch * 8);
+    if (++pc == na + nb) {
+      pc = 0;
+      ++ent;
+    }
+  }
+  *dst = make_uint4(0, 0, 0, 0);
+}
+
 struct PoolFusedArgs {
   const bf16_t* x; int ldx;
   const bf16_t* w1; int ldw1;
@@ -1698,6 +1749,7 @@
   float* out; int ld_out;
   const int32_t* needed;
   int n, L, N, q;
+  int zero_x_reach;
 };
 
 template <int KS>
@@ -1711,7 +1763,8 @@
   static constexpr int PART = BIAS + 1024;
   static constexpr int RED = PART + 2 * NW * 32 * 4;
   static constexpr int LIST = RED + 2 * NW * NCOL * 4;
-  static constexpr int STEADY = PW + 2 * (S + 2);
+  static constexpr int STORES = S + 2 + PoolFillCfg::Z;
+  static constexpr int STEADY = PW + 2 * STORES;
   static_assert(STEADY <= 62, "vmcnt is a 6-bit counter");
 };
 
@@ -1734,10 +1787,16 @@
 
   const int G = gridDim.x, b0 = blockIdx.x;
   int nsteps = b0 < a.n ? (a.n - b0 + G - 1) / G : 0;
+  int* myFill = sList + (a.n + G - 1) / G + 8 + wid * pool_fill_cap<NW>(a.n, G);
+  int nfill = 0, fent = 0, fpc = 0;
+  const PoolFillDst fdst = {const_cast<bf16_t*>(a.x), a.ldx, N >> 3, nullptr, 0, 0, L};
+  uint4* dump_g = g_nt_dump + wid * 64 + lane;
   if (a.needed != nullptr) {
     __shared__ int sCnt[NW + 1];
     const int cand = nsteps;
     const int run = pool_balanced_walk<NW>(a.needed, a.n, G, b0, sList, sCnt, wid, lane);
+    if (a.zero_x_reach >= 0)
+      nfill = pool_fill_list<NW>(a.needed, a.n, G, b0, cand, a.zero_x_reach, myFill, wid, lane, [](bool near) { return near ? 1 : 0; });
     for (int c = wid; c < cand; c += NW) {
       const int sq = b0 + c * G;
       if (a.needed[sq] != 0) continue;
@@ -1748,7 +1807,10 @@
   } else {
     for (int c = tid; c < nsteps; c += 512) sList[c] = b0 + c * G;
   }
-  if (nsteps == 0) return;
+  if (nsteps == 0) {
+    while (fent < nfill) pool_fill_store(myFill, nfill, fent, fpc, fdst, lane, dump_g);
+    return;
+  }
 
   const int wcol0 = wid * TPW * 16;
   bf16x8 bfr[TPW][KS];
@@ -1790,7 +1852,6 @@
       }
     }
   };
-  uint4* dump_g = g_nt_dump + wid * 64 + lane;
   const int offA = fr * 64 + ((g ^ swzP(fr)) << 4);
   const int cc = lane, ccp = cc >> 2, ccs = cc & 3;
   const bool cc_ok = cc * 8 < N;
@@ -1910,9 +1971,11 @@
 #pragma unroll 1
   for (int k = 0; k < nsteps + 2; ++k) {
     if (k >= 2) asm volatile("s_waitcnt vmcnt(%0)" ::"n"(Cfg::STEADY) : "memory");
-    else wait_vmcnt_le(k == 0 ? (NS - 3) * PW : PW + (Cfg::S + 2));
+    else wait_vmcnt_le(k == 0 ? (NS - 3) * PW : PW + Cfg::STORES);
     __builtin_amdgcn_s_barrier();
     issue_stage(k + NS - 2);
+#pragma unroll
+    for (int z = 0; z < PoolFillCfg::Z; ++z) pool_fill_store(myFill, nfill, fent, fpc, fdst, lane, dump_g);
     if (wid < NW / 2) {
       phase_gemm(k);
       phase_out(k);
@@ -1923,6 +1986,7 @@
       phase_gemm(k);
     }
   }
+  while (fent < nfill) pool_fill_store(myFill, nfill, fent, fpc, fdst, lane, dump_g);
 }
 
 struct PoolFusedBwdArgs {
@@ -1946,7 +2010,7 @@
   static constexpr int EPIECES = RT * KS2, GPIECES = 2, PIECES = EPIECES + GPIECES;
   static constexpr int PW = (PIECES + NW - 1) / NW, STAGE = PIECES * 1024, NS = 5;
   static constexpr int LOADS = 5;
-  static constexpr int OPS = PW + LOADS + 2 + RT * 2;
+  static constexpr int OPS = PW + LOADS + 2 + RT * 2 + PoolFillCfg::Z;
   static constexpr int STEADY = 2 * OPS - PW;
   static constexpr int DUMP = NS * STAGE;
   static constexpr int PARTA = DUMP + NW * 1024;
@@ -1971,42 +2035,26 @@
   float* sPartA = reinterpret_cast<float*>(smem + Cfg::PARTA);
   float* sAlpha = reinterpret_cast<float*>(smem + Cfg::ALPHA);
   float* sW2 = reinterpret_cast<float*>(smem + Cfg::W2);
-  float* sRedW = sW2 + 256;
   int* sList = reinterpret_cast<int*>(smem + Cfg::LIST);
 
   const int G = gridDim.x, b0 = blockIdx.x;
   int nsteps = b0 < a.n ? (a.n - b0 + G - 1) / G : 0;
+  int* myFill = sList + (a.n + G - 1) / G + 8 + wid * pool_fill_cap<NW>(a.n, G);
+  int nfill = 0;
   if (a.nz != nullptr) {
     __shared__ int sCnt[NW + 1];
     const int cand = nsteps;
     const int run = pool_balanced_walk<NW>(a.nz, a.n, G, b0, sList, sCnt, wid, lane);
-    for (int c = wid; c < cand; c += NW) {
-      const int sq = b0 + c * G;
-      if (a.nz[sq] != 0) continue;
-      bool near = false;
-      for (int t = max(0, sq - reach) + lane; t <= min(a.n - 1, sq + reach); t += 64) near |= a.nz[t] != 0;
-      near = __ballot(near) != 0ull;
-      const size_t r0 = (size_t)sq * L;
-      const int xc = N >> 3;
-      if (near || !a.dx_far_unwritten)
-        for (int u = lane; u < L * xc; u += 64) {
-          const int row = u / xc, ch = u - row * xc;
-          *reinterpret_cast<uint4*>(a.dx + (r0 + row) * a.lddx + ch * 8) = make_uint4(0, 0, 0, 0);
-        }
-      if (near)
-        for (int u = lane; u < L * qc; u += 64) {
-          const int row = u / qc, ch = u - row * qc;
-          *reinterpret_cast<uint4*>(a.dpre + (r0 + row) * a.ldp + ch * 8) = make_uint4(0, 0, 0, 0);
-        }
-    }
+    const int lvl = a.dx_far_unwritten;
+    nfill = pool_fill_list<NW>(a.nz, a.n, G, b0, cand, reach, myFill, wid, lane,
+                               [&](bool near) { return ((lvl == 0 || (lvl == 1 && near)) ? 1 : 0) | (near ? 2 : 0); });
     nsteps = run;
   } else {
     for (int c = tid; c < nsteps; c += 512) sList[c] = b0 + c * G;
   }
-  for (int c = tid; c < 256; c += 512) {
-    sW2[c] = c < q ? a.w2[c] : 0.f;
-    sRedW[c] = 0.f;
-  }
+  const PoolFillDst fdst = {a.dx, a.lddx, N >> 3, a.dpre, a.ldp, qc, L};
+  int fent = 0, fpc = 0;
+  for (int c = tid; c < 256; c += 512) sW2[c] = c < q ? a.w2[c] : 0.f;
   const int wcol0 = wid * TPW * 16;
   bf16x8 bfr[TPW][KS2];
 #pragma unroll
@@ -2018,13 +2066,14 @@
   __builtin_amdgcn_s_waitcnt(0x0F70);
   __syncthreads();
   float* prow_out = a.partial + (size_t)blockIdx.x * (q + 1);
+  uint4* dump_g = g_nt_dump + wid * 64 + lane;
   if (nsteps == 0) {
     for (int c = tid; c <= q; c += 512) prow_out[c] = 0.f;
+    while (fent < nfill) pool_fill_store(myFill, nfill, fent, fpc, fdst, lane, dump_g);
     return;
   }
 
   const uint32_t dump_lds = lds0 + Cfg::DUMP + wid * 1024;
-  uint4* dump_g = g_nt_dump + wid * 64 + lane;
   auto issue_stage = [&](int kk) {
     const uint32_t slot = lds0 + (kk % NS) * STAGE;
     const bool real = kk < nsteps;
@@ -2109,6 +2158,8 @@
     else wait_vmcnt_le(k == 0 ? PW + Cfg::LOADS : Cfg::OPS + Cfg::LOADS);
     __builtin_amdgcn_s_barrier();
     issue_stage(k + 2);
+#pragma unroll
+    for (int z = 0; z < PoolFillCfg::Z; ++z) pool_fill_store(myFill, nfill, fent, fpc, fdst, lane, dump_g);
     auto phase_a = [&]()     {
       const bool real = k < nsteps;
       const float* grow = reinterpret_cast<const float*>(smem + (k % NS) * STAGE + EPIECES * 1024);
@@ -2228,12 +2279,14 @@
       phase_b();
     }
   }
-#pragma unroll
-  for (int j = 0; j < 2; ++j)
-#pragma unroll
-    for (int e2 = 0; e2 < 8; ++e2) atomicAdd(sRedW + bcc[j] * 8 + e2, myacc[j * 4096 + e2]);
+  while (fent < nfill) pool_fill_store(myFill, nfill, fent, fpc, fdst, lane, dump_g);
   __syncthreads();
-  for (int c = tid; c < q; c += 512) prow_out[c] = sRedW[c];
+  const float* accs = reinterpret_cast<const float*>(smem + Cfg::ACCW);
+  for (int c = tid; c < q; c += 512) {
+    float v = 0.f;
+    for (int u = c >> 3; u < L * qc; u += qc) v += accs[(u >> 9) * 4096 + (u & 511) * 8 + (c & 7)];
+    prow_out[c] = v;
+  }
   if (tid == 0) prow_out[q] = accb;
 }
 
@@ -3144,7 +3197,7 @@
 
 int nr_launch_pool_fused_fwd(const void* x, int ldx, const void* w1, int ldw1, const float* b1, const float* w2, const float* b2,
                              const float* mask, void* e, int lde, float* alpha, float* out, int ld_out, int n, int L, int N, int q,
-                             const int32_t* needed, hipStream_t stream) {
+                             const int32_t* needed, hipStream_t stream, int x_zero_near) {
   constexpr int KS = 13;
   using Cfg = PoolFusedCfg<KS>;
   NR_CHECK_ARG(nr_pool_fused_fwd_ok(NR_BF16, n, L, N, q, ldw1) && ldx >= N && ldx % 8 == 0 && lde >= q && lde % 8 == 0 &&
@@ -3159,11 +3212,13 @@
   }
   const int grid = n < cus ? n : cus;
   const int max_steps = (n + grid - 1) / grid;
-  const size_t smem = (size_t)Cfg::LIST + (size_t)(max_steps + 8) * sizeof(int);
+  NR_CHECK_ARG(!x_zero_near || needed != nullptr, "pool_fused_fwd: x_zero_near needs the seq_needed flags");
+  const size_t smem = (size_t)Cfg::LIST + 2 * (size_t)(max_steps + 8) * sizeof(int);
   NR_CHECK_ARG(smem <= 160 * 1024, "pool_fused_fwd: %d sequences per workgroup do not fit the LDS list", max_steps);
   PoolFusedArgs a;
   a.x = (const bf16_t*)x; a.ldx = ldx; a.w1 = (const bf16_t*)w1; a.ldw1 = ldw1; a.b1 = b1; a.w2 = w2; a.b2 = b2;
   a.e = (bf16_t*)e; a.lde = lde; a.alpha = alpha; a.out = out; a.ld_out = ld_out; a.needed = needed; a.n = n; a.L = L; a.N = N; a.q = q;
+  a.zero_x_reach = x_zero_near ? 32 / L + 2 : -1;
   auto kern = pool_fused_fwd_kernel<KS>;
   NR_CHECK_HIP(hipFuncSetAttribute(reinterpret_cast<const void*>(kern), hipFuncAttributeMaxDynamicSharedMemorySize, (int)smem));
   NrProfScope ps(stream, needed ? "pool_fused_fwd_needed[bf16,n=%d,L=%d,N=%d,q=%d]" : "pool_fused_fwd[bf16,n=%d,L=%d,N=%d,q=%d]", n, L, N, q);
@@ -3196,12 +3251,12 @@
   int grid = n < cus ? n : cus;
   if (grid > partial_rows) grid = partial_rows;
   const int max_steps = (n + grid - 1) / grid;
-  const size_t smem = (size_t)Cfg::LIST + (size_t)(max_steps + 8) * sizeof(int);
+  const size_t smem = (size_t)Cfg::LIST + 2 * (size_t)(max_steps + 8) * sizeof(int);
   NR_CHECK_ARG(smem <= 160 * 1024, "pool_fused_bwd: %d sequences per workgroup do not fit the LDS list", max_steps);
   PoolFusedBwdArgs a;
   a.x = (const bf16_t*)x; a.ldx = ldx; a.e = (const bf16_t*)e; a.lde = lde; a.alpha = alpha; a.g = g; a.ldg = ldg; a.w2 = w2;
   a.w1t = (const bf16_t*)w1t; a.ldw1t = ldw1t; a.dpre = (bf16_t*)dpre; a.ldp = ldp; a.dx = (bf16_t*)dx; a.lddx = lddx; a.partial = partial;
-  a.nz = nz; a.n = n; a.L = L; a.N = N; a.q = q; a.dx_far_unwritten = (nz != nullptr && dx_far_unwritten) ? 1 : 0;
+  a.nz = nz; a.n = n; a.L = L; a.N = N; a.q = q; a.dx_far_unwritten = (nz != nullptr && dx_far_unwritten) ? (dx_far_unwritten == 2 ? 2 : 1) : 0;
   auto kern = pool_fused_bwd_kernel<KS, KS2>;
   NR_CHECK_HIP(hipFuncSetAttribute(reinterpret_cast<const void*>(kern), hipFuncAttributeMaxDynamicSharedMemorySize, (int)smem));
   NrProfScope ps(stream, "pool_fused_bwd[bf16,n=%d,L=%d,N=%d,q=%d]", n, L, N, q);
@@ -3522,12 +3577,14 @@
   for (int c = threadIdx.x; c < chunks16; c += 256) p[c] = make_uint4(0, 0, 0, 0);
 }
 }
-int nr_launch_needed_list(const int32_t* flags, int n, int32_t* out, void* y, size_t seq_bytes, hipStream_t stream, int reach, bool zeroed) {
+int nr_launch_needed_list(const int32_t* flags, int n, int32_t* out, void* y, size_t seq_bytes, hipStream_t stream, int reach, bool zeroed,
+                          bool fill) {
   NR_CHECK_ARG(flags != nullptr && out != nullptr && y != nullptr && seq_bytes % 16 == 0 && (((uintptr_t)y) & 15) == 0, "needed_list: bad arguments");
   if (!zeroed) NR_CHECK_HIP(hipMemsetAsync(out, 0, 4 * sizeof(int32_t), stream));
   NrProfScope ps(stream, "needed_list[n=%d]", n);
   hipLaunchKernelGGL(needed_list_kernel, dim3((n + 255) / 256), dim3(256), 0, stream, flags, n, out, out + 4);
-  hipLaunchKernelGGL(zero_unneeded_kernel, dim3(n), dim3(256), 0, stream, flags, reinterpret_cast<uint4*>(y), (int)(seq_bytes / 16), n, reach);
+  if (fill)
+    hipLaunchKernelGGL(zero_unneeded_kernel, dim3(n), dim3(256), 0, stream, flags, reinterpret_cast<uint4*>(y), (int)(seq_bytes / 16), n, reach);
   NR_CHECK_LAUNCH();
   return NR_OK;
 }
diff --git a/newsrecommendation_amd/model/NRMS.py b/newsrecommendation_amd/model/NRMS.py
--- a/newsrecommendation_amd/model/NRMS.py
+++ b/newsrecommendation_amd/model/NRMS.py
@@ -26,9 +26,11 @@
         needed = ops.needed_flags(needed)
         far = needed is not None and ops.pool_contracts_slabs(x.shape[0], x.shape[1], self.attn.att_fc1.in_features,
                                                               self.attn.att_fc1.out_features, ops.dtype_code(self.attn.compute_dtype))
+        fill = far and ops.pool_fills_x_zeros(x.shape[0], x.shape[1], self.attn.att_fc1.in_features, self.attn.att_fc1.out_features,
+                                              ops.dtype_code(self.attn.compute_dtype), mask)
         y = self.multi_head_self_attn.forward_gather(x, self.embedding_matrix.weight, mask=mask, p_in=p, p_out=p, needed=needed,
-                                                     far_unwritten=far)
-        return self.attn(y, mask, needed=needed, lazy_dx=far and getattr(y, "_nr_takes_lazy_dy", False))
+                                                     far_unwritten=far, zeros_deferred=fill)
+        return self.attn(y, mask, needed=needed, lazy_dx=far and getattr(y, "_nr_takes_lazy_dy", False), fill_zeros=fill)
 
 
 class UserEncoder(nn.Module):
diff --git a/newsrecommendation_amd/model/model_utils.py b/newsrecommendation_amd/model/model_utils.py
--- a/newsrecommendation_amd/model/model_utils.py
+++ b/newsrecommendation_amd/model/model_utils.py
@@ -12,13 +12,15 @@
         self.att_fc2 = nn.Linear(hidden_size, 1)
         self.compute_dtype = compute_dtype
 
-    def forward(self, x, attn_mask=None, needed=None, lazy_dx=False):
+    def forward(self, x, attn_mask=None, needed=None, lazy_dx=False, fill_zeros=False):
         code = ops.dtype_code(self.compute_dtype)
         if x.dtype != ops.torch_dtype(code):
+            if fill_zeros:
+                raise RuntimeError("fill_zeros: x must be the MHSA output itself, in the compute dtype")
             x = ops.to_compute(x.float(), code)
             lazy_dx = False
         return ops.additive_pool(x, self.att_fc1.weight, self.att_fc1.bias, self.att_fc2.weight, self.att_fc2.bias,
-                                 code, mask=attn_mask, needed=needed, lazy_dx=lazy_dx)
+                                 code, mask=attn_mask, needed=needed, lazy_dx=lazy_dx, fill_zeros=fill_zeros)
 
 
 class ScaledDotProductAttention(nn.Module):
@@ -66,7 +68,8 @@
         return ops.mhsa(x, *self._params(), heads=self.n_heads, code=code, mask=mask, p_out=p_out,
                         flat=getattr(self, "_nr_flat", None))
 
-    def forward_gather(self, ids, table, mask=None, p_in=0.0, p_out=0.0, needed=None, far_unwritten=False):
+    def forward_gather(self, ids, table, mask=None, p_in=0.0, p_out=0.0, needed=None, far_unwritten=False, zeros_deferred=False):
         code = ops.dtype_code(self.compute_dtype)
         return ops.mhsa(None, *self._params(), heads=self.n_heads, code=code, mask=mask, ids=ids, table=table,
-                        p_in=p_in, p_out=p_out, flat=getattr(self, "_nr_flat", None), needed=needed, far_unwritten=far_unwritten)
+                        p_in=p_in, p_out=p_out, flat=getattr(self, "_nr_flat", None), needed=needed, far_unwritten=far_unwritten,
+                        zeros_deferred=zeros_deferred)
diff --git a/newsrecommendation_amd/ops.py b/newsrecommendation_amd/ops.py
--- a/newsrecommendation_amd/ops.py
+++ b/newsrecommendation_amd/ops.py
@@ -333,6 +333,7 @@
                           mask=ptr(mask_c), w_qkv=ptr(w_p), ldw=w_p.shape[1], b_qkv=ptr(b_p),
                           x_rows=ptr(x_rows), ld_rows=Kp, seq_needed=ptr(cfg.get("needed")),
                           y_far_unwritten=int(bool(cfg.get("far_unwritten")) and cfg.get("needed") is not None),
+                          y_zeros_deferred=int(bool(cfg.get("zeros_deferred")) and bool(cfg.get("far_unwritten")) and cfg.get("needed") is not None),
                           table_rows=cfg["table_shape"][0] if gather else 0)
         row_ws = _ws(_lib.lib().nr_mhsa_workspace_bytes(C.byref(d)), dev) if keep_rows and code == _lib.NR_BF16 else None
         d.row_ws, d.row_ws_bytes = ptr(row_ws), (row_ws.numel() * 4 if row_ws is not None else 0)
@@ -438,11 +439,17 @@
     return bool(_lib.lib().nr_pool_contracts_slabs(C.byref(d)))
 
 
+def pool_fills_x_zeros(n: int, L: int, N: int, q: int, code: int, mask=None) -> bool:
+    d = _lib.PoolDesc(n=int(n), L=int(L), N=int(N), q=int(q), dtype=int(code), mask=ptr(mask),
+                      ldw1=round_up(int(N), 32 if code == NR_BF16 else chunk(code)))
+    return bool(_lib.lib().nr_pool_fills_x_zeros(C.byref(d)))
+
+
 def mhsa(x, wq, bq, wk, bk, wv, bv, heads: int, code: int, mask=None, ids=None, table=None, p_in=0.0, p_out=0.0, flat=None,
-         needed=None, far_unwritten=False):
+         needed=None, far_unwritten=False, zeros_deferred=False):
     cfg = dict(code=code, heads=heads, p_in=float(p_in), p_out=float(p_out),
                seed_in=draw_seed() if p_in > 0 else 0, seed_out=draw_seed() if p_out > 0 else 0, needed=needed,
-               far_unwritten=bool(far_unwritten))
+               far_unwritten=bool(far_unwritten), zeros_deferred=bool(zeros_deferred))
     if flat is not None:
         cfg["flat"] = flat
     if ids is not None:
@@ -545,7 +552,7 @@
 class PoolFunction(Function):
 
     @staticmethod
-    def forward(ctx, x, w1, b1, w2, b2, mask, code, needed=None, lazy_dx=False):
+    def forward(ctx, x, w1, b1, w2, b2, mask, code, needed=None, lazy_dx=0, fill_zeros=False):
         _need_gpu(x, w1, mask)
         n, L, N = x.shape
         q = w1.shape[0]
@@ -560,11 +567,11 @@
         alpha = torch.empty(n * L, dtype=torch.float32, device=dev)
         out = torch.empty(n, N, dtype=torch.float32, device=dev)
         d = _lib.PoolDesc(n=n, L=L, N=N, q=q, dtype=code, x=ptr(x), mask=ptr(mask_c), w1=ptr(w1_p), ldw1=w1_p.shape[1],
-                          b1=ptr(b1_c), w2=ptr(w2_c), b2=ptr(b2_c), seq_needed=ptr(needed))
+                          b1=ptr(b1_c), w2=ptr(w2_c), b2=ptr(b2_c), seq_needed=ptr(needed), x_zero_near=int(bool(fill_zeros)))
         check(_lib.lib().nr_additive_pool_fwd(C.byref(d), ptr(e), ptr(alpha), ptr(out), N, _stream()), "nr_additive_pool_fwd")
         ctx.code, ctx.dims = code, (n, L, N, q)
         ctx.needed = needed
-        ctx.lazy_dx = bool(lazy_dx)
+        ctx.lazy_dx = int(lazy_dx)
         ctx.targets = tuple(grad_target(p) for p in (w1, b1, w2, b2))
         ctx.save_for_backward(x, mask_c, w1_p, b1_c, w2_c, b2_c, e, alpha, w1)
         return out
@@ -586,21 +593,22 @@
             dw1, db1, dw2, db2 = flat[:q * N].view(q, N), flat[q * N:q * N + q], flat[q * N + q:q * N + 2 * q], flat[q * N + 2 * q:q * N + 2 * q + 1]
         dx = torch.empty_like(x) if ctx.needs_input_grad[0] else None
         d = _lib.PoolDesc(n=n, L=L, N=N, q=q, dtype=code, x=ptr(x), mask=ptr(mask_c), w1=ptr(w1_p), ldw1=w1_p.shape[1],
-                          b1=ptr(b1_c), w2=ptr(w2_c), b2=ptr(b2_c), seq_needed=ptr(ctx.needed), dx_far_unwritten=int(ctx.lazy_dx))
+                          b1=ptr(b1_c), w2=ptr(w2_c), b2=ptr(b2_c), seq_needed=ptr(ctx.needed), dx_far_unwritten=ctx.lazy_dx)
         partial = _ws(_lib.lib().nr_pool_workspace_bytes(C.byref(d)), dev)
         d.partial_bytes = partial.numel() * 4
         check(_lib.lib().nr_additive_pool_bwd(C.byref(d), ptr(e), ptr(alpha), ptr(g), N, ptr(w1_t),
                                               w1_t.shape[1] if w1_t is not None else 0, ptr(dpre), ptr(partial), ptr(dw1),
                                               ptr(db1), ptr(dw2), ptr(db2), ptr(dx), _stream()), "nr_additive_pool_bwd")
         flags_ptr = _lib.lib().nr_pool_seq_flags(C.byref(d), ptr(partial))
-        _offer_flags(seq, dx, n, flags_ptr, partial, lazy=ctx.lazy_dx and bool(flags_ptr))
+        _offer_flags(seq, dx, n, flags_ptr, partial, lazy=bool(ctx.lazy_dx) and bool(flags_ptr))
         if direct:
-            return dx, None, None, None, None, None, None, None, None
-        return dx, dw1, db1, dw2.view(1, q), db2, None, None, None, None
-
-
-def additive_pool(x, w1, b1, w2, b2, code: int, mask=None, needed=None, lazy_dx=False):
-    return PoolFunction.apply(x, w1, b1, w2, b2, mask, code, needed, bool(lazy_dx) and x.requires_grad)
+            return dx, None, None, None, None, None, None, None, None, None
+        return dx, dw1, db1, dw2.view(1, q), db2, None, None, None, None, None
+
+
+def additive_pool(x, w1, b1, w2, b2, code: int, mask=None, needed=None, lazy_dx=False, fill_zeros=False):
+    level = (2 if getattr(x, "_nr_takes_lazy_dy", False) else 1) if (lazy_dx and x.requires_grad) else 0
+    return PoolFunction.apply(x, w1, b1, w2, b2, mask, code, needed, level, bool(fill_zeros) and needed is not None)
 
 
 _grad_out = {}
```

After: 175,400 impressions/s (median of 6 runs). Within noise of the previous version (+0.9%).
